# silencht/SG-SLAM

Hardware: AMD Instinct MI355X
Metric: tracked frames/sec (640x480 RGB-D) (higher is better)
Workload: dtype u8/f32(bf16x3 matrix products)/f64

## Files before the change

### include/sgx_debug.h

```cpp
#ifndef SGX_DEBUG_H
#define SGX_DEBUG_H
#include "sgx.h"
#ifdef __cplusplus
extern "C" {
#endif

int sgx_orb_debug_level_geometry(const sgx_orb *h, int level, int32_t *w, int32_t *hgt, int32_t *stride);
int sgx_orb_debug_set_unfused_pyramid(int on);
int sgx_orb_debug_read_level(sgx_orb *h, int frame, int level, uint8_t *dst );
int sgx_orb_debug_read_candidates(sgx_orb *h, int frame, int level, int32_t *x, int32_t *y, int32_t *score, int cap, int *n);
int sgx_debug_flow_affine_batch_dev(int batch, int cap, const sgx_keypoint *d_keys, const int32_t *d_n, const float *d_A, const float *d_shift, const float *d_boxes,
                                    int max_boxes, float *d_prev_xy, void *stream);
int sgx_pose_opt_debug_set_threads(int threads_per_frame);
int sgx_ba_debug_last_plan(int32_t plan[4]);
int sgx_ba_debug_set_init(int mode);
int sgx_ba_debug_set_jobs(int host);
int sgx_ba_debug_set_solver(int mode);
int sgx_det_debug_read_blob(sgx_det *h, const char *blob_name, int image, float *dst, int cap, int *n);
int sgx_flow_debug_read_level(sgx_flow *h, int slot, int frame, int level, uint8_t *img);
int sgx_flow_debug_level_size(const sgx_flow *h, int level, int32_t *w, int32_t *hgt);
int sgx_pnp_debug_betas(int which, const double *L, const double *rho, double *betas);
int sgx_debug_corun_bf16(int blocks, int iters, int launches, void *stream);
int sgx_det_debug_detection_output(sgx_det *h, const float *loc, const float *conf, int batch, sgx_det_result *results);
int sgx_det_debug_continued(sgx_det *h, int *count);
int sgx_det_debug_set_fusion(int on);
int sgx_det_debug_set_irb(int on);
int sgx_det_debug_set_block_fusion(int on);
int sgx_det_debug_set_gemm(int mode);
int sgx_det_debug_set_legacy_kernels(int on);
int sgx_det_debug_time_ops(sgx_det *h, const uint8_t *d_img, int pitch, int batch, int reps, float *ms, int cap, int *nops);
int sgx_det_debug_run_step(sgx_det *h, const uint8_t *d_img, int pitch, int batch, int step, int reps, void *stream);
int sgx_orb_debug_run_octree(sgx_orb *h, int level, const uint32_t *packed, int n, uint32_t *out_sel, int cap, int *nsel);

#ifdef __cplusplus
}
#endif
#endif
```

### sg_slam_amd/capi.py

```python
import ctypes as C
import numpy as np

KP_DTYPE = np.dtype([('x', 'f4'), ('y', 'f4'), ('size', 'f4'), ('angle', 'f4'), ('response', 'f4'),
                     ('octave', 'i4'), ('class_id', 'i4')])


class SgxError(RuntimeError):
    pass


class Camera(C.Structure):
    _fields_ = [('fx', C.c_float), ('fy', C.c_float), ('cx', C.c_float), ('cy', C.c_float), ('bf', C.c_float),
                ('min_x', C.c_float), ('max_x', C.c_float), ('min_y', C.c_float), ('max_y', C.c_float)]


class BaProblem(C.Structure):
    _fields_ = [('n_poses', C.c_int32), ('n_points', C.c_int32), ('n_edges', C.c_int32), ('poses', C.c_void_p), ('pose_fixed', C.c_void_p),
                ('points', C.c_void_p), ('edge_pose', C.c_void_p), ('edge_point', C.c_void_p), ('edge_obs', C.c_void_p), ('edge_info', C.c_void_p)]


class BaStats(C.Structure):
    _fields_ = [('iterations_first', C.c_int32), ('iterations_second', C.c_int32), ('free_poses', C.c_int32), ('reserved', C.c_int32),
                ('chi2_first', C.c_double), ('chi2_second', C.c_double)]


SGX_DET_MAX = 100


class Detection(C.Structure):
    _fields_ = [(k, C.c_float) for k in ('label', 'score', 'xmin', 'ymin', 'xmax', 'ymax')]


class Object2D(C.Structure):
    _fields_ = [('id', C.c_int32)] + [(k, C.c_float) for k in ('prob', 'x', 'y', 'w', 'h')]


class DetResult(C.Structure):
    _fields_ = [('n_raw', C.c_int32), ('raw', Detection * SGX_DET_MAX), ('n_objects', C.c_int32), ('objects', Object2D * SGX_DET_MAX),
                ('have_dynamic_for_mapping', C.c_int32), ('have_dynamic_for_rm_feature', C.c_int32),
                ('n_map_boxes', C.c_int32), ('map_boxes', Object2D * SGX_DET_MAX), ('n_rm_boxes', C.c_int32), ('rm_boxes', Object2D * SGX_DET_MAX)]


class FlowConfig(C.Structure):
    _fields_ = [('width', C.c_int32), ('height', C.c_int32), ('max_batch', C.c_int32), ('win_size', C.c_int32), ('max_level', C.c_int32),
                ('max_count', C.c_int32), ('epsilon', C.c_double)]


class TrackerConfig(C.Structure):
    _fields_ = [('streams', C.c_int32), ('width', C.c_int32), ('height', C.c_int32), ('nfeatures', C.c_int32), ('scale_factor', C.c_float), ('nlevels', C.c_int32),
                ('ini_th_fast', C.c_int32), ('min_th_fast', C.c_int32), ('cam', Camera), ('depth_map_factor', C.c_float), ('th_projection', C.c_float),
                ('local_map', C.c_int32), ('dynamic_mask', C.c_int32), ('max_boxes', C.c_int32), ('pipelined', C.c_int32)]


class OrbConfig(C.Structure):
    _fields_ = [('nfeatures', C.c_int32), ('scale_factor', C.c_float), ('nlevels', C.c_int32),
                ('ini_th_fast', C.c_int32), ('min_th_fast', C.c_int32), ('width', C.c_int32),
                ('height', C.c_int32), ('max_batch', C.c_int32)]


SYMBOLS = [
    'sgx_version', 'sgx_status_string', 'sgx_orb_create', 'sgx_orb_destroy', 'sgx_orb_keypoint_capacity', 'sgx_orb_get_tables',
    'sgx_orb_extract_batch_dev', 'sgx_orb_extract', 'sgx_orb_last_status', 'sgx_profile_enable', 'sgx_profile_num_classes', 'sgx_profile_class_name',
    'sgx_profile_read', 'sgx_match_project_frame_batch_dev', 'sgx_match_project_frame', 'sgx_match_project_local_batch_dev',
    'sgx_match_project_local', 'sgx_frame_stereo_from_rgbd_batch_dev', 'sgx_frame_unproject_batch_dev', 'sgx_frame_make_map_points_batch_dev',
    'sgx_frame_merge_matches_batch_dev', 'sgx_pose_optimization_batch_dev', 'sgx_pose_optimization', 'sgx_frame_motion_model_batch_dev',
    'sgx_local_bundle_adjustment', 'sgx_bundle_adjustment', 'sgx_det_create', 'sgx_det_destroy', 'sgx_det_info', 'sgx_det_detect',
    'sgx_det_detect_batch_dev', 'sgx_det_forward_batch_dev', 'sgx_frame_compact_keys_batch_dev', 'sgx_frame_gray_from_color_batch_dev',
    'sgx_det_gemm_mode', 'sgx_det_plan_step', 'sgx_dynamic_mask_batch_dev', 'sgx_tracker_create', 'sgx_tracker_destroy',
    'sgx_tracker_keypoint_capacity', 'sgx_tracker_record_bytes', 'sgx_tracker_set_initial_pose', 'sgx_tracker_step_dev', 'sgx_tracker_host_buffers',
    'sgx_tracker_step_host', 'sgx_tracker_wait_inputs', 'sgx_tracker_sync', 'sgx_tracker_read', 'sgx_tracker_snapshot_pose_dev',
    'sgx_tracker_snapshot_boxes_dev', 'sgx_tracker_pack_records_dev', 'sgx_tracker_frame_dev', 'sgx_tracker_extractor', 'sgx_flow_create',
    'sgx_dist_unique_id', 'sgx_dist_create', 'sgx_dist_destroy', 'sgx_dist_world', 'sgx_dist_gather_records',
    'sgx_flow_destroy', 'sgx_flow_reset', 'sgx_flow_levels', 'sgx_flow_lk_batch_dev', 'sgx_flow_lk', 'sgx_fundamental_ransac_batch_dev',
    'sgx_find_fundamental_mat', 'sgx_hamming_matrix', 'sgx_hamming_matrix_dev', 'sgx_match_search_for_triangulation', 'sgx_match_search_by_bow',
    'sgx_match_search_by_bow_kf', 'sgx_match_fuse_search', 'sgx_match_project_keyframe', 'sgx_match_fuse_search_sim3',
    'sgx_triangulate_new_map_points', 'sgx_mappoint_update_normal_and_depth', 'sgx_mappoint_distinctive_descriptors', 'sgx_sim3_solver_create',
    'sgx_sim3_solver_set_ransac_parameters', 'sgx_sim3_solver_iterate', 'sgx_sim3_solver_get_estimate', 'sgx_sim3_solver_destroy',
    'sgx_match_search_for_initialization', 'sgx_voc_load', 'sgx_voc_create', 'sgx_voc_info', 'sgx_voc_destroy', 'sgx_voc_transform',
    'sgx_voc_transform_batch_dev', 'sgx_voc_score', 'sgx_match_project_sim3', 'sgx_match_search_by_sim3', 'sgx_optimize_sim3',
    'sgx_optimize_essential_graph', 'sgx_correct_map_points', 'sgx_undistort_points', 'sgx_frame_undistort_stereo_rgbd_batch_dev', 'sgx_frame_image_bounds',
    'sgx_tracker_set_distortion', 'sgx_tracker_frame_keys_un_dev', 'sgx_pnp_solver_create', 'sgx_pnp_solver_set_ransac_parameters', 'sgx_pnp_solver_iterate',
    'sgx_pnp_solver_get_estimate', 'sgx_pnp_solver_destroy', 'sgx_pnp_batch_create', 'sgx_pnp_batch_set_dev', 'sgx_pnp_batch_iterate_dev', 'sgx_pnp_batch_destroy',
]
TAP_SYMBOLS = [
    'sgx_orb_debug_level_geometry', 'sgx_orb_debug_set_unfused_pyramid', 'sgx_orb_debug_read_level', 'sgx_orb_debug_read_candidates',
    'sgx_orb_debug_run_octree', 'sgx_pose_opt_debug_set_threads', 'sgx_ba_debug_set_solver', 'sgx_ba_debug_set_jobs', 'sgx_ba_debug_set_init', 'sgx_ba_debug_last_plan', 'sgx_det_debug_read_blob',
    'sgx_det_debug_detection_output', 'sgx_det_debug_continued', 'sgx_debug_flow_affine_batch_dev', 'sgx_det_debug_set_fusion', 'sgx_det_debug_set_legacy_kernels',
    'sgx_det_debug_set_block_fusion', 'sgx_det_debug_set_irb', 'sgx_det_debug_set_gemm', 'sgx_det_debug_time_ops', 'sgx_det_debug_run_step', 'sgx_flow_debug_read_level',
    'sgx_flow_debug_level_size', 'sgx_debug_corun_bf16', 'sgx_pnp_debug_betas',
]


def _vp(x):
    if x is None:
        return None
    if isinstance(x, int):
        return C.c_void_p(x)
    if hasattr(x, 'data_ptr'):
        return C.c_void_p(x.data_ptr())
    return x.ctypes.data_as(C.c_void_p)


class SgxLib:
    def __init__(self, path):
        self.path = path
        self.dll = C.CDLL(path)
        d = self.dll
        d.sgx_version.restype = C.c_char_p
        d.sgx_status_string.restype = C.c_char_p
        d.sgx_status_string.argtypes = [C.c_int]
        d.sgx_orb_create.argtypes = [C.POINTER(OrbConfig), C.POINTER(C.c_void_p)]
        d.sgx_orb_destroy.argtypes = [C.c_void_p]
        d.sgx_orb_destroy.restype = None
        d.sgx_orb_keypoint_capacity.argtypes = [C.c_void_p]
        d.sgx_orb_get_tables.argtypes = [C.c_void_p] + [C.c_void_p] * 5
        d.sgx_orb_extract_batch_dev.argtypes = [C.c_void_p, C.c_void_p, C.c_int, C.c_int, C.c_void_p, C.c_void_p,
                                                C.c_void_p, C.c_int, C.c_void_p]
        d.sgx_orb_extract.argtypes = [C.c_void_p, C.c_void_p, C.c_int, C.c_void_p, C.c_void_p, C.c_int, C.POINTER(C.c_int)]
        d.sgx_orb_last_status.argtypes = [C.c_void_p, C.c_void_p]

        d.sgx_profile_enable.argtypes = [C.c_int]
        d.sgx_profile_class_name.restype = C.c_char_p
        d.sgx_profile_class_name.argtypes = [C.c_int]
        d.sgx_profile_read.argtypes = [C.c_void_p, C.c_void_p, C.c_int]

        vp = C.c_void_p
        d.sgx_match_project_frame_batch_dev.argtypes = [C.c_int, C.c_int] + [vp] * 13 + [C.POINTER(Camera), vp, C.c_int, C.c_float, C.c_int, C.c_int, vp, vp, vp]
        d.sgx_match_project_frame.argtypes = [C.c_int] + [vp] * 4 + [C.c_int] + [vp] * 7 + [C.POINTER(Camera), vp, C.c_int, C.c_float, C.c_int, C.c_int, vp, vp]
        d.sgx_frame_stereo_from_rgbd_batch_dev.argtypes = [C.c_int, C.c_int, vp, vp, vp, C.c_int, C.c_int, C.c_float, C.c_float, vp, vp, vp]
        d.sgx_frame_unproject_batch_dev.argtypes = [C.c_int, C.c_int, vp, vp, vp, vp, C.POINTER(Camera), vp, vp, vp]
        d.sgx_pose_optimization_batch_dev.argtypes = [C.c_int, C.c_int, vp, vp, vp, vp, vp, vp, C.c_int, vp, C.c_int, C.POINTER(Camera), vp, vp, vp, vp]
        d.sgx_pose_optimization.argtypes = [C.c_int, vp, vp, vp, vp, vp, C.c_int, C.POINTER(Camera), vp, vp, vp]
        d.sgx_frame_motion_model_batch_dev.argtypes = [C.c_int, vp, vp, vp, vp, vp]
        d.sgx_local_bundle_adjustment.argtypes = [C.POINTER(BaProblem), C.POINTER(Camera), vp, vp, C.POINTER(BaStats)]
        d.sgx_bundle_adjustment.argtypes = [C.POINTER(BaProblem), C.POINTER(Camera), C.c_int, vp, C.c_int, C.POINTER(BaStats)]
        d.sgx_det_create.argtypes = [C.c_char_p, vp, C.c_size_t, C.c_int, C.c_int, C.c_int, C.c_float, C.c_float, C.POINTER(vp)]
        d.sgx_det_destroy.argtypes = [vp]; d.sgx_det_destroy.restype = None
        d.sgx_det_info.argtypes = [vp, C.POINTER(C.c_int32), C.POINTER(C.c_int32), C.POINTER(C.c_int32), C.POINTER(C.c_double)]
        d.sgx_det_detect.argtypes = [vp, vp, C.c_int, C.c_int, C.POINTER(DetResult)]
        d.sgx_det_detect_batch_dev.argtypes = [vp, vp, C.c_int, C.c_int, vp, vp, vp, C.c_int, vp, vp]
        d.sgx_det_forward_batch_dev.argtypes = [vp, vp, C.c_int, C.c_int, C.POINTER(vp), C.POINTER(vp), vp]
        d.sgx_det_gemm_mode.argtypes = [vp]
        d.sgx_tracker_create.argtypes = [C.POINTER(TrackerConfig), vp, C.POINTER(vp)]
        d.sgx_tracker_destroy.argtypes = [vp]; d.sgx_tracker_destroy.restype = None
        d.sgx_tracker_keypoint_capacity.argtypes = [vp]
        d.sgx_tracker_record_bytes.argtypes = [vp]
        d.sgx_tracker_set_initial_pose.argtypes = [vp, vp]
        d.sgx_tracker_step_dev.argtypes = [vp, vp, C.c_int, vp, vp, C.c_int, vp]
        d.sgx_tracker_host_buffers.argtypes = [vp, C.c_int, C.POINTER(vp), C.POINTER(C.c_int), C.POINTER(vp)]
        d.sgx_tracker_step_host.argtypes = [vp, C.c_int, C.c_int]
        d.sgx_tracker_sync.argtypes = [vp]
        d.sgx_tracker_wait_inputs.argtypes = [vp, C.c_int]
        d.sgx_tracker_read.argtypes = [vp] * 10
        d.sgx_tracker_snapshot_pose_dev.argtypes = [vp, vp]
        d.sgx_tracker_snapshot_boxes_dev.argtypes = [vp, C.c_int, vp, vp]
        d.sgx_tracker_pack_records_dev.argtypes = [vp, vp, vp]
        d.sgx_dist_unique_id.argtypes = [vp]
        d.sgx_dist_create.argtypes = [vp, C.c_int, C.c_int, C.POINTER(vp)]
        d.sgx_dist_destroy.argtypes = [vp]; d.sgx_dist_destroy.restype = None
        d.sgx_dist_world.argtypes = [vp, C.POINTER(C.c_int32), C.POINTER(C.c_int32)]
        d.sgx_dist_gather_records.argtypes = [vp, vp, C.c_size_t, vp, C.c_int, vp]
        d.sgx_tracker_frame_dev.argtypes = [vp] + [C.POINTER(vp)] * 6
        d.sgx_tracker_extractor.argtypes = [vp]; d.sgx_tracker_extractor.restype = vp
        d.sgx_det_plan_step.argtypes = [vp, C.c_int, C.c_char_p, C.c_int]
        d.sgx_dynamic_mask_batch_dev.argtypes = [C.c_int, C.c_int, vp, vp, vp, vp, vp, vp, C.c_int, vp, vp]
        d.sgx_frame_gray_from_color_batch_dev.argtypes = [C.c_int, C.c_int, C.c_int, vp, C.c_int, C.c_int, C.c_int, vp, C.c_int, vp]
        d.sgx_frame_compact_keys_batch_dev.argtypes = [C.c_int, C.c_int, vp, vp, vp, vp, vp, C.c_int, vp, vp, vp, vp]
        d.sgx_match_project_local.argtypes = [C.c_int] + [vp] * 5 + [C.c_int] + [vp] * 7 + [C.POINTER(Camera), vp, C.c_int, C.c_float, C.c_float, C.c_float, C.c_float, vp, vp, vp]
        d.sgx_match_project_local_batch_dev.argtypes = [C.c_int, C.c_int] + [vp] * 6 + [C.c_int] + [vp] * 8 + [C.POINTER(Camera), vp, C.c_int, C.c_float, C.c_float, C.c_float, C.c_float, vp, vp, vp, vp]
        d.sgx_undistort_points.argtypes = [C.c_int, vp, vp, vp, C.c_int, vp]
        d.sgx_frame_undistort_stereo_rgbd_batch_dev.argtypes = [C.c_int, C.c_int, vp, vp, vp, C.c_int, C.POINTER(Camera), vp, C.c_int, C.c_int, C.c_float, vp, vp, vp, vp]
        d.sgx_frame_image_bounds.argtypes = [C.c_int, C.c_int, vp, vp, C.c_int, C.POINTER(Camera)]
        d.sgx_tracker_set_distortion.argtypes = [vp, vp, C.c_int, C.POINTER(Camera)]
        d.sgx_tracker_frame_keys_un_dev.argtypes = [vp, C.POINTER(vp)]
        d.sgx_frame_make_map_points_batch_dev.argtypes = [C.c_int, C.c_int, C.c_int] + [vp] * 7 + [C.c_int] + [vp] * 7
        d.sgx_frame_merge_matches_batch_dev.argtypes = [C.c_int, C.c_int] + [vp] * 10
        d.sgx_flow_create.argtypes = [C.POINTER(FlowConfig), C.POINTER(vp)]
        d.sgx_flow_destroy.argtypes = [vp]; d.sgx_flow_destroy.restype = None
        d.sgx_flow_reset.argtypes = [vp]
        d.sgx_flow_levels.argtypes = [vp]
        d.sgx_flow_lk_batch_dev.argtypes = [vp, vp, C.c_int, C.c_int, vp, vp, C.c_int, vp, vp, C.POINTER(C.c_int32), vp]
        d.sgx_flow_lk.argtypes = [vp, vp, vp, C.c_int, vp, C.c_int, vp, vp]
        d.sgx_fundamental_ransac_batch_dev.argtypes = [C.c_int, C.c_int] + [vp] * 6 + [C.c_int, C.c_double, C.c_double, vp, vp, vp, vp]
        d.sgx_find_fundamental_mat.argtypes = [vp, vp, C.c_int, C.c_double, C.c_double, vp, vp, vp]
        d.sgx_hamming_matrix.argtypes = [vp, C.c_int, vp, C.c_int, vp]
        d.sgx_optimize_essential_graph.argtypes = [C.c_int, vp, vp, C.c_int, vp, vp, vp, C.c_int, C.c_int, vp, vp]
        d.sgx_correct_map_points.argtypes = [C.c_int, vp, vp, C.c_int, vp, vp, vp]
        d.sgx_optimize_sim3.argtypes = [C.c_int] + [vp] * 9 + [C.c_float, C.c_int, vp, vp, vp]
        d.sgx_match_project_keyframe.argtypes = [C.c_int] + [vp] * 4 + [C.c_int] + [vp] * 6 + [C.POINTER(Camera), vp, C.c_int, C.c_float, C.c_float, C.c_int, C.c_int, vp, vp]
        d.sgx_match_search_by_bow.argtypes = [C.c_int] + [vp] * 4 + [C.c_int] + [vp] * 3 + [C.c_float, C.c_int, vp, vp]
        d.sgx_match_fuse_search_sim3.argtypes = [C.c_int, vp, vp, vp, C.c_int] + [vp] * 6 + [vp, vp, C.c_int, C.c_float, C.c_float, vp, vp, vp]
        d.sgx_match_project_sim3.argtypes = [C.c_int, vp, vp, vp, vp, C.c_int] + [vp] * 6 + [vp, vp, C.c_int, C.c_float, C.c_int, vp, vp]
        d.sgx_match_search_by_sim3.argtypes = ([C.c_int] + [vp] * 8) * 2 + [vp, vp, C.c_int, C.c_float, C.c_float, vp, vp, C.c_float, vp, vp]
        d.sgx_match_search_for_initialization.argtypes = [C.c_int, vp, vp, C.c_int, vp, vp, vp, C.c_int, C.c_float, C.c_int, vp, vp, vp]
        d.sgx_sim3_solver_create.argtypes = [C.c_int] + [vp] * 6 + [C.c_int, C.c_uint, vp]
        d.sgx_sim3_solver_set_ransac_parameters.argtypes = [vp, C.c_double, C.c_int, C.c_int]
        d.sgx_sim3_solver_iterate.argtypes = [vp, C.c_int] + [vp] * 7
        d.sgx_sim3_solver_get_estimate.argtypes = [vp] * 5
        d.sgx_sim3_solver_destroy.argtypes = [vp]; d.sgx_sim3_solver_destroy.restype = None
        d.sgx_pnp_solver_create.argtypes = [C.c_int] + [vp] * 4 + [C.c_uint, vp]
        d.sgx_pnp_solver_set_ransac_parameters.argtypes = [vp, C.c_double, C.c_int, C.c_int, C.c_int, C.c_float, C.c_float]
        d.sgx_pnp_solver_iterate.argtypes = [vp, C.c_int] + [vp] * 7
        d.sgx_pnp_solver_get_estimate.argtypes = [vp] * 6
        d.sgx_pnp_solver_destroy.argtypes = [vp]; d.sgx_pnp_solver_destroy.restype = None
        d.sgx_pnp_batch_create.argtypes = [C.c_int, C.c_int, vp]
        d.sgx_pnp_batch_set_dev.argtypes = [vp, C.c_int] + [vp] * 8
        d.sgx_pnp_batch_iterate_dev.argtypes = [vp, C.c_int, vp, C.c_int, vp, vp, vp, vp]
        d.sgx_pnp_batch_destroy.argtypes = [vp]; d.sgx_pnp_batch_destroy.restype = None
        d.sgx_mappoint_update_normal_and_depth.argtypes = [C.c_int] + [vp] * 6 + [C.c_int, vp, vp, vp]
        d.sgx_mappoint_distinctive_descriptors.argtypes = [C.c_int, vp, vp, vp, vp]
        d.sgx_triangulate_new_map_points.argtypes = [C.c_int, vp] + [C.c_int] + [vp] * 5 + [C.c_int] + [vp] * 5 + [vp, vp, vp, C.c_int, vp, vp, vp]
        d.sgx_voc_load.argtypes = [C.c_char_p, vp]
        d.sgx_voc_create.argtypes = [C.c_int] * 5 + [vp] * 5
        d.sgx_voc_info.argtypes = [vp] * 7
        d.sgx_voc_destroy.argtypes = [vp]; d.sgx_voc_destroy.restype = None
        d.sgx_voc_transform.argtypes = [vp, C.c_int, vp, C.c_int, vp, vp, vp, vp, vp]
        d.sgx_voc_transform_batch_dev.argtypes = [vp, vp, C.c_size_t, vp, C.c_int, C.c_int, C.c_int, vp, vp, vp, vp]
        d.sgx_voc_score.argtypes = [vp, C.c_int, vp, vp, C.c_int, vp, vp, vp]
        d.sgx_match_search_by_bow_kf.argtypes = [C.c_int] + [vp] * 4 + [C.c_int] + [vp] * 4 + [C.c_float, C.c_int, vp, vp]
        d.sgx_match_fuse_search.argtypes = [C.c_int] + [vp] * 4 + [C.c_int] + [vp] * 6 + [C.POINTER(Camera), vp, vp, C.c_int, C.c_float, C.c_float, vp, vp, vp]
        d.sgx_hamming_matrix_dev.argtypes = [vp, C.c_int, vp, C.c_int, vp, vp]
        d.sgx_match_search_for_triangulation.argtypes = [C.c_int] + [vp] * 6 + [C.c_int] + [vp] * 6 + [vp, C.POINTER(Camera), vp, vp, C.c_int, C.c_int, C.c_int, vp, vp]

        self.has_taps = hasattr(d, 'sgx_det_debug_read_blob')
        if self.has_taps:
            d.sgx_orb_debug_level_geometry.argtypes = [C.c_void_p, C.c_int] + [C.POINTER(C.c_int32)] * 3
            d.sgx_orb_debug_read_level.argtypes = [C.c_void_p, C.c_int, C.c_int, C.c_void_p]
            d.sgx_orb_debug_read_candidates.argtypes = [C.c_void_p, C.c_int, C.c_int, C.c_void_p, C.c_void_p, C.c_void_p, C.c_int, C.POINTER(C.c_int)]
            d.sgx_orb_debug_run_octree.argtypes = [C.c_void_p, C.c_int, C.c_void_p, C.c_int, C.c_void_p, C.c_int, C.POINTER(C.c_int)]
            d.sgx_orb_debug_set_unfused_pyramid.argtypes = [C.c_int]
            d.sgx_pose_opt_debug_set_threads.argtypes = [C.c_int]
            d.sgx_ba_debug_set_solver.argtypes = [C.c_int]
            d.sgx_ba_debug_set_jobs.argtypes = [C.c_int]
            d.sgx_ba_debug_set_init.argtypes = [C.c_int]
            d.sgx_ba_debug_last_plan.argtypes = [C.c_void_p]
            d.sgx_det_debug_detection_output.argtypes = [vp, vp, vp, C.c_int, C.POINTER(DetResult)]
            d.sgx_det_debug_continued.argtypes = [vp, C.POINTER(C.c_int)]
            d.sgx_det_debug_read_blob.argtypes = [vp, C.c_char_p, C.c_int, vp, C.c_int, C.POINTER(C.c_int)]
            for nm in ('fusion', 'legacy_kernels', 'block_fusion', 'irb', 'gemm'):
                getattr(d, 'sgx_det_debug_set_' + nm).argtypes = [C.c_int]
            d.sgx_det_debug_time_ops.argtypes = [vp, vp, C.c_int, C.c_int, C.c_int, vp, C.c_int, C.POINTER(C.c_int)]
            d.sgx_det_debug_run_step.argtypes = [vp, vp, C.c_int, C.c_int, C.c_int, C.c_int, vp]
            d.sgx_debug_flow_affine_batch_dev.argtypes = [C.c_int, C.c_int, vp, vp, vp, vp, vp, C.c_int, vp, vp]
            d.sgx_flow_debug_read_level.argtypes = [vp, C.c_int, C.c_int, C.c_int, vp]
            d.sgx_debug_corun_bf16.argtypes = [C.c_int, C.c_int, C.c_int, vp]
            d.sgx_pnp_debug_betas.argtypes = [C.c_int, vp, vp, vp]
            d.sgx_flow_debug_level_size.argtypes = [vp, C.c_int, C.POINTER(C.c_int32), C.POINTER(C.c_int32)]

    def tap(self, name):
        if not self.has_taps:
            raise SgxError(f'{name}: {self.path} is the product build and has no test taps; use tests/taps/libsgx_taps.so (make -C sg_slam_amd/csrc taps)')
        return getattr(self.dll, name)

    def version(self):
        return self.dll.sgx_version().decode()

    def check(self, rc, what=''):
        if rc != 0:
            raise SgxError(f'{what}: {self.dll.sgx_status_string(rc).decode()} ({rc})')

    def profile_enable(self, on=True):
        self.check(self.dll.sgx_profile_enable(int(on)))

    def profile_read(self, reset=True):
        n = self.dll.sgx_profile_num_classes()
        ms = np.zeros(n, 'f4'); cnt = np.zeros(n, 'i4')
        self.check(self.dll.sgx_profile_read(_vp(ms), _vp(cnt), int(reset)), 'sgx_profile_read')
        return {self.dll.sgx_profile_class_name(k).decode(): (float(ms[k]), int(cnt[k])) for k in range(n)}
```

### sg_slam_amd/csrc/sgx_det.cpp

```cpp
#include "sgx_block.h"
#include "sgx_det_block.h"
#include "sgx_det_irb.h"
#include "sgx_det_bf16.h"
#include "sgx_det_hrb.h"
#include "sgx_prof.h"
#include "../../include/sgx.h"
#ifdef SGX_DEBUG_TAPS
#include "../../include/sgx_debug.h"
#endif
#include <math.h>
#include <stdio.h>
#include <stdlib.h>
#include <string.h>
#include <algorithm>
#include <map>
#include <memory>
#include <sstream>
#include <string>
#include <vector>


namespace {
struct Layer {
    std::string type, name;
    std::vector<std::string> ins, outs;
    std::map<int, double> p;
    std::map<int, std::vector<float>> pa;
    int geti(int k, int d) const { auto it = p.find(k); return it == p.end() ? d : (int)it->second; }
    float getf(int k, float d) const { auto it = p.find(k); return it == p.end() ? d : (float)it->second; }
};
struct Blob { int c = 0, h = 0, w = 0; size_t n = 0; float *d = nullptr; bool scalar = false; float sval = 0.f; int alias = -1; };
enum OpKind { OP_PW, OP_KXK, OP_BINARY, OP_UNARY, OP_PERMUTE_INTO, OP_COPY_INTO, OP_SOFTMAX, OP_FUSED_BLOCK, OP_IRB, OP_SE_GATE };
struct EpiStep { int op, src; float a, b; int tensor; };
struct Op {
    OpKind kind; int in0 = -1, in1 = -1, out = -1;
    std::vector<EpiStep> epi; int hwc = 0, hwc_off = 0; bool dead = false; std::string name;
    int inc = 0, outc = 0, H = 0, W = 0, Ho = 0, Wo = 0, k = 1, stride = 1, pad = 0, depthwise = 0, act = 0; float lo = 0, hi = 0;
    std::vector<float> hw, hb;
    float *wt = nullptr, *bias = nullptr, *wtT = nullptr, *wtP = nullptr; int ldw = 0;
    int bop = 0; int off = 0; int rows = 0, C = 0;
    void *wS = nullptr;
    int res_blob = -1;
    SgxFusedBlk fb;
    SgxSeGate sg;
    SgxIrb irb; int irb_out2_blob = -1;
};
}

#ifndef SGX_DET_GRAPH_EXECS
#define SGX_DET_GRAPH_EXECS 1
#endif
#ifndef SGX_DET_FORK_LANES
#define SGX_DET_FORK_LANES 1
#endif

#ifndef SGX_DET_GEMM_DEFAULT
#define SGX_DET_GEMM_DEFAULT 1
#endif
struct DetSwitches {
    int fuse = 1, legacy = 0, block_fusion = 0;
    int irb = 1;
    int gemm = SGX_DET_GEMM_DEFAULT;
    int block2 = 1, block2_se = 1, hrb = 1, hrb_pick = 0, fb2_tile = -1, fb_dbg = 0;
    int irb_mask = 0xff;
    int irb_g = 0, irb_nbuf = 0, irb_split = 0, irb_minhw = 0, irb_stagger = 1, irb_w1lds = 0, irb3 = 0, irb3_dbg = 0, irb_a3 = 0, irb_dual = 1, se_gate = 1;
    int prefuse = 1, xcd = 1;
    int stem_words = 13824, dw2 = 1, dw3 = 0, dw_budget = 8192, pw3_mink = 64, pw3_force = 0, pw2_direct = 1;
    int no_graph = 0, fork_lanes = SGX_DET_FORK_LANES, graph_execs = SGX_DET_GRAPH_EXECS, skip_output = 0;
    int out_single = 0;
};

struct sgx_det {
    int T = 300, max_batch = 1, W = 0, H = 0;
    int pre_fused = 0;
    DetSwitches sw;
    float det_th = 0.9f, dyn_th = 0.01f;
    std::vector<Layer> layers;
    std::map<std::string, int> blob_id;
    std::vector<Blob> blobs;
    std::vector<Op> ops;
    std::vector<void *> dev;
    std::vector<float> priors;
    int num_priors = 0, num_class = 21, nms_top_k = 300, keep_top_k = 100; float nms_th = 0.45f, conf_th = 0.01f, dvar[4] = {0.1f, 0.1f, 0.2f, 0.2f};
    int loc_blob = -1, conf_blob = -1;
    SgxDetTab *d_xt = nullptr, *d_yt = nullptr; uint8_t *d_img = nullptr;
    float *d_priors = nullptr, *d_cls_rows = nullptr; int *d_cls_count = nullptr; sgx_det_result *d_results = nullptr;
    int *d_cls_ncut = nullptr, *d_cls_cont = nullptr; uint32_t *d_cls_next = nullptr, *d_sstar = nullptr;
    int last_out_batch = 0;
    double gmac = 0;
#ifndef SGX_EMU
    std::map<int, std::vector<hipGraphExec_t>> graphs;
    std::map<int, unsigned> graph_turn;
    std::vector<hipStream_t> fork_streams;
    std::vector<hipEvent_t> fork_events;
#endif
    ~sgx_det() {
#ifndef SGX_EMU
        for (auto &g : graphs) for (hipGraphExec_t e : g.second) (void)hipGraphExecDestroy(e);
        for (hipEvent_t e : fork_events) (void)hipEventDestroy(e);
        for (hipStream_t q : fork_streams) (void)hipStreamDestroy(q);
#endif
        for (void *p : dev) (void)hipFree(p);
    }
    template <class Tp> int alloc(Tp **p, size_t n) { void *q = nullptr; if (hipMalloc(&q, (n ? n : 1) * sizeof(Tp)) != hipSuccess) return SGX_ERR_NOMEM; dev.push_back(q); *p = (Tp *)q; return SGX_OK; }
    template <class Tp, class Pp> int upload(Pp *dst, const Tp *src, size_t n) { Tp *d = nullptr; if (alloc(&d, n)) return SGX_ERR_NOMEM; *dst = (Pp)d; return hipMemcpy(d, src, n * sizeof(Tp), hipMemcpyHostToDevice) == hipSuccess ? SGX_OK : SGX_ERR_DEVICE; }
    template <class Tp, class Pp> int upload(Pp *dst, const std::vector<Tp> &v) { return upload(dst, v.data(), v.size()); }
    int resolve(int id) const { while (blobs[id].alias >= 0) id = blobs[id].alias; return id; }
    bool is_output(int id) const { return id == loc_blob || id == conf_blob; }
};

static thread_local int g_det_fuse = 1, g_det_block_fusion = 0, g_det_legacy = 0;
static thread_local int g_det_irb = -1, g_det_gemm = -1;
SGX_TAP int sgx_det_debug_set_fusion(int on) { g_det_fuse = on ? 1 : 0; return SGX_OK; }
SGX_TAP int sgx_det_debug_set_legacy_kernels(int on) { g_det_legacy = on ? 1 : 0; return SGX_OK; }
SGX_TAP int sgx_det_debug_set_block_fusion(int on) { g_det_block_fusion = on ? 1 : 0; return SGX_OK; }
SGX_TAP int sgx_det_debug_set_irb(int on) { g_det_irb = on < 0 ? -1 : (on > 2 ? 2 : on); return SGX_OK; }
SGX_TAP int sgx_det_debug_set_gemm(int mode) { g_det_gemm = mode < 0 ? -1 : (mode ? 1 : 0); return SGX_OK; }
extern "C" int sgx_det_gemm_mode(const sgx_det *h) { return h ? h->sw.gemm : -1; }

static DetSwitches det_switches()
{
    auto env = [](const char *name, int &v) { if (const char *e = sgx_getenv(name)) v = atoi(e); };
    DetSwitches s;
    s.fuse = g_det_fuse; s.legacy = g_det_legacy; s.block_fusion = (g_det_block_fusion || sgx_getenv("SGX_DET_BLOCK_FUSION")) ? 1 : 0;
    env("SGX_DET_IRB", s.irb); if (g_det_irb >= 0) s.irb = g_det_irb;
#ifdef SGX_EMU
    s.gemm = 0;
#endif
    if (const char *e = sgx_getenv("SGX_DET_GEMM")) if (*e) s.gemm = (!strcmp(e, "f32") || !strcmp(e, "0")) ? 0 : 1;
    if (g_det_gemm >= 0) s.gemm = g_det_gemm;
    if (s.legacy) s.gemm = 0;
    env("SGX_DET_BLOCK2", s.block2); env("SGX_DET_BLOCK2_SE", s.block2_se); env("SGX_DET_HRB", s.hrb); env("SGX_HRB_PICK", s.hrb_pick); env("SGX_FB2_TILE", s.fb2_tile); env("SGX_FB_DBG", s.fb_dbg);
    env("SGX_DET_IRB_MASK", s.irb_mask); env("SGX_IRB_G", s.irb_g); env("SGX_IRB_NBUF", s.irb_nbuf); env("SGX_IRB_SPLIT", s.irb_split); env("SGX_IRB_MINHW", s.irb_minhw);
    env("SGX_IRB_STAGGER", s.irb_stagger); env("SGX_IRB_W1LDS", s.irb_w1lds); env("SGX_DET_IRB3", s.irb3); env("SGX_IRB3_DBG", s.irb3_dbg); env("SGX_DET_IRB_A3", s.irb_a3);
    env("SGX_DET_IRB_DUAL", s.irb_dual); env("SGX_DET_SE_GATE", s.se_gate); env("SGX_DET_PREFUSE", s.prefuse); env("SGX_DET_XCD", s.xcd);
    env("SGX_DET_STEM_WORDS", s.stem_words); env("SGX_DW2", s.dw2); env("SGX_DW3", s.dw3); env("SGX_DW_BUDGET", s.dw_budget);
    env("SGX_PW3_MINK", s.pw3_mink); env("SGX_PW3_FORCE", s.pw3_force); env("SGX_PW2_DIRECT", s.pw2_direct);
    s.no_graph = sgx_getenv("SGX_DET_NO_GRAPH") != nullptr; env("SGX_DET_FORK", s.fork_lanes); env("SGX_DET_EXECS", s.graph_execs);
    s.skip_output = sgx_getenv("SGX_DET_SKIP_OUTPUT") != nullptr;
    s.out_single = sgx_getenv("SGX_DET_OUT_SINGLE") != nullptr;
    return s;
}

struct Stem2Geom { int nbx4, pitch4, RB, nbands; size_t lds; };
static Stem2Geom stem2_geom(const sgx_det *h, const Op &op)
{
    Stem2Geom g;
    g.nbx4 = (op.Wo + 3) / 4; g.pitch4 = ((g.nbx4 - 1) * 4 * op.stride + 3 * op.stride + op.k + 3) & ~3;
    const int words = h->sw.stem_words;
    g.RB = std::max(1, std::min(op.Ho, ((words / (3 * g.pitch4)) - 3) / 2 + 1));
    g.nbands = (op.Ho + g.RB - 1) / g.RB;
    g.lds = (size_t)3 * ((g.RB - 1) * 2 + 3) * g.pitch4 * 4;
    return g;
}
static SgxEpi make_epi(const sgx_det *h, const Op &op, size_t tpitch);
static bool stem2_ok(const sgx_det *h, const Op &op)
{
    if (op.kind != OP_KXK || !h->sw.dw2 || h->sw.legacy || op.depthwise || !op.wtT || op.outc > 16 || op.inc != 3 || op.k != 3 || op.stride != 2) return false;
    const Stem2Geom g = stem2_geom(h, op);
    if (!(3 * 5 * g.pitch4 * 4 <= 65536 && g.pitch4 < 4096)) return false;
    const int mode = make_epi(h, op, 0).mode;
    return mode == SGX_EMODE_NONE || mode == SGX_EMODE_ACT || mode == SGX_EMODE_HSWISH;
}

static int parse_param(const char *text, std::vector<Layer> &layers)
{
    std::istringstream is(text);
    std::string line;
    if (!std::getline(is, line) || atoi(line.c_str()) != 7767517) return SGX_ERR_INVALID;
    if (!std::getline(is, line)) return SGX_ERR_INVALID;
    while (std::getline(is, line)) {
        std::istringstream ls(line);
        Layer L; int nin = 0, nout = 0;
        if (!(ls >> L.type >> L.name >> nin >> nout)) continue;
        for (int i = 0; i < nin; i++) { std::string s; ls >> s; L.ins.push_back(s); }
        for (int i = 0; i < nout; i++) { std::string s; ls >> s; L.outs.push_back(s); }
        std::string kv;
        while (ls >> kv) {
            const size_t eq = kv.find('=');
            if (eq == std::string::npos) continue;
            const int k = atoi(kv.substr(0, eq).c_str());
            const std::string v = kv.substr(eq + 1);
            if (k <= -23300) {
                std::vector<float> arr; std::istringstream vs(v); std::string tok; bool first = true;
                while (std::getline(vs, tok, ',')) { if (first) { first = false; continue; } arr.push_back((float)atof(tok.c_str())); }
                L.pa[-k - 23300] = arr;
            } else L.p[k] = atof(v.c_str());
        }
        layers.push_back(L);
    }
    return layers.empty() ? SGX_ERR_INVALID : SGX_OK;
}

static void build_tab(int s, int d, std::vector<SgxDetTab> &t)
{
    t.resize(d);
    const double scale = (double)s / d;
    for (int i = 0; i < d; i++) {
        float f = (float)((i + 0.5) * scale - 0.5);
        int si = (int)floorf(f); f -= si;
        if (si < 0) { si = 0; f = 0.f; }
        if (si >= s - 1) { si = s - 2; f = 1.f; }
        t[i].o = (short)si; t[i].a0 = (short)lrintf((1.f - f) * 2048); t[i].a1 = (short)lrintf(f * 2048); t[i].pad = 0;
    }
}

extern "C" void sgx_det_destroy(sgx_det *h) { delete h; }

namespace {
struct Loader {
    sgx_det *h; const uint8_t *bp; size_t bin_bytes, bo = 0;
    std::vector<float> prior_boxes, prior_vars;
    int blob(const std::string &n) { auto it = h->blob_id.find(n); if (it != h->blob_id.end()) return it->second; h->blob_id[n] = (int)h->blobs.size(); h->blobs.push_back(Blob()); return (int)h->blobs.size() - 1; }
    void same_shape_op(Op &op, const Layer &L, const Blob &A) { const int oid = blob(L.outs[0]); Blob &ob = h->blobs[oid]; ob = A; ob.alias = -1; ob.d = nullptr; op.out = oid; op.name = L.name; h->ops.push_back(op); }
    int conv(const Layer &L, int in0, const Blob &A);
    void priorbox(const Layer &L, const Blob &A);
    int run();
};

std::vector<float> pair_interleave(const std::vector<float> &w, int C, int kk)
{
    std::vector<float> p((size_t)C * kk); for (int m = 0; m < C; m++) for (int t = 0; t < kk; t++) p[((size_t)(m >> 1) * kk + t) * 2 + (m & 1)] = w[(size_t)m * kk + t]; return p;
}
int upload_se_interleaved(sgx_det *h, const Op &d, const Op &e, const float **wq1p, const float **wq2p)
{
    const int Cq = d.outc, Co = d.inc;
    std::vector<float> p1((size_t)Cq * Co), p2((size_t)Co * Cq);
    for (int j = 0; j < Cq; j++) for (int k = 0; k < Co; k++) p1[((size_t)(j >> 1) * Co + k) * 2 + (j & 1)] = d.hw[(size_t)j * Co + k];
    for (int co = 0; co < Co; co++) for (int j = 0; j < Cq; j++) p2[((size_t)j * (Co / 2) + (co >> 1)) * 2 + (co & 1)] = e.hw[(size_t)co * Cq + j];
    const int rc = h->upload(wq1p, p1);
    return rc ? rc : h->upload(wq2p, p2);
}

int Loader::conv(const Layer &L, int in0, const Blob &A)
{
    Op op; const int outc = L.geti(0, 0), k = L.geti(1, 1), stride = L.geti(3, 1), pad = L.geti(4, 0), wsize = L.geti(6, 0), group = L.geti(7, 1);
    const int inc = A.c;
    if (L.geti(2, 1) != 1 || (group != 1 && group != inc) || wsize != outc * (inc / group) * k * k) return SGX_ERR_UNSUPPORTED;
    if (bo + 4 + (size_t)wsize * 4 + (L.geti(5, 0) ? (size_t)outc * 4 : 0) > bin_bytes) return SGX_ERR_INVALID;
    uint32_t flag; memcpy(&flag, bp + bo, 4); bo += 4;
    if (flag != 0) return SGX_ERR_UNSUPPORTED;
    op.hw.resize(wsize); memcpy(op.hw.data(), bp + bo, (size_t)wsize * 4); bo += (size_t)wsize * 4;
    op.hb.assign(outc, 0.f);
    if (L.geti(5, 0)) { memcpy(op.hb.data(), bp + bo, (size_t)outc * 4); bo += (size_t)outc * 4; }
    int rc = h->upload(&op.wt, op.hw); if (rc) return rc;
    if ((rc = h->upload(&op.bias, op.hb))) return rc;
    const bool pw = (k == 1 && group == 1 && stride == 1 && pad == 0), stem = (group == 1 && k > 1 && outc <= 16);
    if (pw || stem) {
        const int kk = inc * k * k, ldo = pw ? ((outc + 31) / 32) * 32 + 128 : 16;
        op.ldw = ldo;
        std::vector<float> wT((size_t)(pw ? ((kk + 31) / 32) * 32 : kk) * ldo, 0.f);
        for (int o = 0; o < outc; o++) for (int q = 0; q < kk; q++) wT[(size_t)q * ldo + o] = op.hw[(size_t)o * kk + q];
        if ((rc = h->upload(&op.wtT, wT))) return rc;
        if (pw && h->sw.gemm == 1) {
            std::vector<unsigned short> ws((size_t)((kk + 15) / 16) * 6 * ldo * 8);
            sgx_split_weights_bf16x3(op.hw.data(), outc, kk, ldo, ws.data());
            if ((rc = h->upload(&op.wS, ws))) return rc;
        }
    }
#ifdef SGX_DEBUG_TAPS
    if (group == inc && group != 1 && (outc & 1) == 0 && inc == outc && (rc = h->upload(&op.wtP, pair_interleave(op.hw, outc, k * k)))) return rc;
#endif
    op.inc = inc; op.outc = outc; op.H = A.h; op.W = A.w; op.k = k; op.stride = stride; op.pad = pad; op.depthwise = group != 1;
    op.Ho = (A.h + 2 * pad - k) / stride + 1; op.Wo = (A.w + 2 * pad - k) / stride + 1;
    op.kind = pw ? OP_PW : OP_KXK;
    op.in0 = in0;
    h->gmac += (double)op.Ho * op.Wo * wsize * 1e-9;
    const int oid = blob(L.outs[0]); Blob &ob = h->blobs[oid]; ob = Blob(); ob.c = outc; ob.h = op.Ho; ob.w = op.Wo; ob.n = (size_t)outc * op.Ho * op.Wo;
    op.out = oid; op.name = L.name;
    h->ops.push_back(op);
    return SGX_OK;
}

void Loader::priorbox(const Layer &L, const Blob &A)
{
    const int T = h->T;
    const std::vector<float> mins = L.pa.count(0) ? L.pa.at(0) : std::vector<float>(), maxs = L.pa.count(1) ? L.pa.at(1) : std::vector<float>(), ars = L.pa.count(2) ? L.pa.at(2) : std::vector<float>();
    const int flip = L.geti(7, 1), clip = L.geti(8, 0); const float offset = L.getf(13, 0.f);
    const float step_w = (float)T / (float)A.w, step_h = (float)T / (float)A.h;
    const float var[4] = { L.getf(3, .1f), L.getf(4, .1f), L.getf(5, .2f), L.getf(6, .2f) };
    auto add = [&](float cx, float cy, float bw, float bh) {
        float bx[4] = { (cx - bw * 0.5f) / T, (cy - bh * 0.5f) / T, (cx + bw * 0.5f) / T, (cy + bh * 0.5f) / T };
        for (int q = 0; q < 4; q++) { prior_boxes.push_back(clip ? std::min(std::max(bx[q], 0.f), 1.f) : bx[q]); prior_vars.push_back(var[q]); }
    };
    for (int i = 0; i < A.h; i++) for (int j = 0; j < A.w; j++) {
        const float cx = ((float)j + offset) * step_w, cy = ((float)i + offset) * step_h;
        for (size_t kk = 0; kk < mins.size(); kk++) {
            const float ms = mins[kk]; add(cx, cy, ms, ms);
            if (!maxs.empty()) { const float s = sqrtf(ms * maxs[kk]); add(cx, cy, s, s); }
            for (float ar : ars) { const float sq = sqrtf(ar); add(cx, cy, ms * sq, ms / sq); if (flip) add(cx, cy, ms / sq, ms * sq); }
        }
    }
    blob(L.outs[0]);
}

int Loader::run()
{
    const int B = h->max_batch, T = h->T;
    for (const Layer &L : h->layers) {
        if (L.type == "Input") { Blob &b = h->blobs[blob(L.outs[0])]; b.c = 3; b.h = T; b.w = T; b.n = (size_t)3 * T * T; if (h->alloc(&b.d, b.n * B)) return SGX_ERR_NOMEM; continue; }
        if (L.type == "MemoryData") {
            const int n = L.geti(0, 0) * std::max(L.geti(1, 1), 1) * std::max(L.geti(2, 1), 1);
            if (n != 1 || bo + 4 > bin_bytes) return SGX_ERR_UNSUPPORTED;
            Blob &b = h->blobs[blob(L.outs[0])]; b.scalar = true; memcpy(&b.sval, bp + bo, 4); bo += 4; b.n = 1; continue;
        }
        if (L.type == "Split") { const int src = h->resolve(blob(L.ins[0])); for (const std::string &o : L.outs) { const int id = blob(o); h->blobs[id] = h->blobs[src]; h->blobs[id].alias = src; } continue; }
        const int in0 = h->resolve(blob(L.ins[0]));
        const Blob A = h->blobs[in0];
        if (L.type == "Convolution" || L.type == "ConvolutionDepthWise") { const int rc = conv(L, in0, A); if (rc) return rc; continue; }
        if (L.type == "ReLU" || L.type == "Clip") {
            Op op; op.kind = OP_UNARY; op.in0 = in0; op.act = L.type == "ReLU" ? SGX_ACT_RELU : SGX_ACT_CLIP; op.lo = L.getf(0, 0.f); op.hi = L.getf(1, 0.f);
            same_shape_op(op, L, A); continue;
        }
        if (L.type == "BinaryOp") {
            const int in1 = h->resolve(blob(L.ins[1]));
            Op op; op.kind = OP_BINARY; op.in0 = in0; op.in1 = in1; op.bop = L.geti(0, 0);
            if (op.bop != 0 && op.bop != 2 && op.bop != 3) return SGX_ERR_UNSUPPORTED;
            if (!h->blobs[in1].scalar && h->blobs[in1].n != A.n) return SGX_ERR_UNSUPPORTED;
            same_shape_op(op, L, A); continue;
        }
        const int raw_in = blob(L.ins[0]);
        if (L.type == "Permute") { if (L.geti(0, 0) != 3) return SGX_ERR_UNSUPPORTED; const int oid = blob(L.outs[0]); h->blobs[oid] = A; h->blobs[oid].alias = raw_in; h->blobs[oid].sval = 1.f;  continue; }
        if (L.type == "Flatten") { const int oid = blob(L.outs[0]); h->blobs[oid] = A; h->blobs[oid].sval = 0.f; h->blobs[oid].alias = raw_in; continue; }
        if (L.type == "PriorBox") { priorbox(L, A); continue; }
        if (L.type == "Concat") {
            if (L.name == "mbox_priorbox") { blob(L.outs[0]); continue; }
            size_t total = 0; for (const std::string &i : L.ins) total += h->blobs[h->resolve(blob(i))].n;
            const int oid = blob(L.outs[0]); Blob &ob = h->blobs[oid]; ob.c = 1; ob.h = 1; ob.w = (int)total; ob.n = total;
            int off = 0;
            for (const std::string &i : L.ins) {
                int id = blob(i); bool hwc = false; while (h->blobs[id].alias >= 0) { if (h->blobs[id].sval == 1.f) hwc = true; id = h->blobs[id].alias; }
                Op op; op.kind = hwc ? OP_PERMUTE_INTO : OP_COPY_INTO; op.in0 = id; op.out = oid; op.off = off; op.C = h->blobs[id].c; op.rows = h->blobs[id].h * h->blobs[id].w;
                op.name = L.name; h->ops.push_back(op); off += (int)h->blobs[id].n;
            }
            continue;
        }
        if (L.type == "Reshape") { const int oid = blob(L.outs[0]); h->blobs[oid] = A; h->blobs[oid].alias = raw_in; h->blobs[oid].w = L.geti(0, 1); h->blobs[oid].h = (int)(A.n / L.geti(0, 1)); continue; }
        if (L.type == "Softmax") {
            Op op; op.kind = OP_SOFTMAX; op.in0 = in0; op.C = h->blobs[blob(L.ins[0])].w; op.rows = (int)(A.n / op.C);
            if (op.C < 1 || op.C > SGX_SOFTMAX_MAXC) return SGX_ERR_UNSUPPORTED;
            same_shape_op(op, L, A); continue;
        }
        if (L.type == "DetectionOutput") {
            h->loc_blob = h->resolve(blob(L.ins[0])); h->conf_blob = h->resolve(blob(L.ins[1]));
            h->num_class = L.geti(0, 21); h->nms_th = L.getf(1, 0.45f); h->nms_top_k = L.geti(2, 300); h->keep_top_k = L.geti(3, 100); h->conf_th = L.getf(4, 0.01f);
            h->dvar[0] = L.getf(5, .1f); h->dvar[1] = L.getf(6, .1f); h->dvar[2] = L.getf(7, .2f); h->dvar[3] = L.getf(8, .2f);
            continue;
        }
        return SGX_ERR_UNSUPPORTED;
    }
    if (h->loc_blob < 0 || h->conf_blob < 0) return SGX_ERR_INVALID;
    h->num_priors = (int)prior_boxes.size() / 4;
    h->priors = prior_boxes; h->priors.insert(h->priors.end(), prior_vars.begin(), prior_vars.end());
    return SGX_OK;
}

struct EpiClass { int mode = SGX_EMODE_GENERIC; float c1 = 0.f, lo = 0.f, hi = INFINITY, c2 = 1.f; int i0 = -1, i1 = -1, t0 = -1, t1 = -1; };
template <class Step> EpiClass classify_epi(const Step *e, size_t n)
{
    EpiClass r;
    auto is = [&](size_t i, int opc, int src) { return i < n && e[i].op == opc && (opc == SGX_EOP_CLIP || opc == SGX_EOP_RELU || e[i].src == src); };
    if (n == 0) r.mode = SGX_EMODE_NONE;
    else if (n == 1 && is(0, SGX_EOP_RELU, 0)) { r.mode = SGX_EMODE_ACT; r.lo = 0.f; r.hi = INFINITY; }
    else if (n == 1 && is(0, SGX_EOP_CLIP, 0)) { r.mode = SGX_EMODE_ACT; r.lo = e[0].a; r.hi = e[0].b; }
    else if (n == 1 && is(0, SGX_EOP_ADD, SGX_ESRC_TENSOR)) { r.mode = SGX_EMODE_ADD_T; r.i1 = 0; }
    else if (n == 4 && is(0, SGX_EOP_ADD, SGX_ESRC_CONST) && is(1, SGX_EOP_CLIP, 0) && is(2, SGX_EOP_MUL, SGX_ESRC_ROOT) && is(3, SGX_EOP_DIV, SGX_ESRC_CONST)) {
        r.mode = SGX_EMODE_HSWISH; r.c1 = e[0].a; r.lo = e[1].a; r.hi = e[1].b; r.c2 = e[3].a;
    } else if ((n == 4 || n == 5) && is(0, SGX_EOP_ADD, SGX_ESRC_CONST) && is(1, SGX_EOP_CLIP, 0) && is(2, SGX_EOP_DIV, SGX_ESRC_CONST) && is(3, SGX_EOP_MUL, SGX_ESRC_TENSOR) &&
               (n == 4 || is(4, SGX_EOP_ADD, SGX_ESRC_TENSOR))) {
        r.mode = n == 4 ? SGX_EMODE_GATE : SGX_EMODE_GATE_ADD; r.c1 = e[0].a; r.lo = e[1].a; r.hi = e[1].b; r.c2 = e[2].a; r.i0 = 3; if (n == 5) r.i1 = 4;
    }
    return r;
}
EpiClass classify(const std::vector<EpiStep> &e) { EpiClass r = classify_epi(e.data(), e.size()); if (r.i0 >= 0) r.t0 = e[r.i0].tensor; if (r.i1 >= 0) r.t1 = e[r.i1].tensor; return r; }

SgxFusedBlk make_fused_blk(const Op &a, const Op &bq, const Op &c, const EpiClass &ca, const EpiClass &cb)
{
    SgxFusedBlk fb; memset(&fb, 0, sizeof fb);
    fb.Cin = a.inc; fb.Cmid = a.outc; fb.Cout = c.outc; fb.K = bq.k; fb.stride = bq.stride; fb.pad = bq.pad; fb.H = a.H; fb.W = a.W; fb.Ho = bq.Ho; fb.Wo = bq.Wo;
    fb.lo1 = ca.lo; fb.hi1 = ca.hi; fb.lo2 = cb.lo; fb.hi2 = cb.hi;
    fb.w1 = a.wt; fb.b1 = a.bias; fb.wd = bq.wt; fb.bd = bq.bias; fb.w2 = c.wt; fb.b2 = c.bias;
    return fb;
}
void set_tiles(SgxFusedBlk &fb) { fb.tiles_x = (fb.Wo + fb.TOW - 1) / fb.TOW; fb.tiles_y = (fb.Ho + fb.TOH - 1) / fb.TOH; }
Op make_block_op(const Op &a, const Op &bq, const Op &c, const SgxFusedBlk &fb, int out, int res, const std::string &name)
{
    Op f; f.kind = OP_FUSED_BLOCK; f.in0 = a.in0; f.out = out; f.name = name; f.fb = fb; f.res_blob = res;
    f.inc = a.inc; f.outc = c.outc; f.H = a.H; f.W = a.W; f.Ho = bq.Ho; f.Wo = bq.Wo; f.k = bq.k; f.stride = bq.stride;
    return f;
}

struct Planner {
    sgx_det *h; const DetSwitches &sw; std::vector<Op> &ops; const int nops, B;
    std::vector<int> R;
    explicit Planner(sgx_det *h_) : h(h_), sw(h_->sw), ops(h_->ops), nops((int)h_->ops.size()), B(h_->max_batch) {}
    bool fb2_on() const { return sw.block2 != 0 && !sw.legacy && sw.fuse; }
    void readers(int id, std::vector<int> &r, bool all = false) const
    {
        r.clear();
        for (int i = 0; i < nops; i++) {
            const Op &o = ops[i];
            if (o.dead) continue;
            bool rd = o.in0 == id || (o.kind == OP_BINARY && o.in1 == id && !h->blobs[id].scalar);
            if (all) {
                rd = rd || o.res_blob == id;
                for (const EpiStep &st : o.epi) rd = rd || st.tensor == id;
            }
            if (rd) r.push_back(i);
        }
    }
    void readers_all(int id, std::vector<int> &r) const { readers(id, r, true); }
    int fuse_epilogues(), fuse_blocks(), fuse_irb(), fuse_se_gates(), merge_dual_heads();
    int fuse_block_fb1(int ai, int bi, int ci, const EpiClass &ca, const EpiClass &cb, int res);
    struct IrbMatch { int ai = -1, bi = -1, ci = -1, di = -1, ei = -1, out_blob = -1, res_blob = -1; EpiClass ca, cb, cc, cd, ce; };
    bool match_irb(int bi, IrbMatch &m);
    int fuse_block2_se(const IrbMatch &m, bool *taken);
    bool irb_geometry(const IrbMatch &m, SgxIrb &ib) const;
};

int Planner::fuse_epilogues()
{
    std::vector<int> producer(h->blobs.size(), -2);
    producer[h->resolve(h->blob_id.at("input"))] = -1;
    for (int i = 0; i < nops; i++) if (ops[i].kind != OP_PERMUTE_INTO && ops[i].kind != OP_COPY_INTO) producer[ops[i].out] = i;
    for (int ci = 0; ci < nops; ci++) {
        Op &cv = ops[ci];
        if (cv.kind != OP_PW && cv.kind != OP_KXK) continue;
        const int root = cv.out;
        int cur = root, root_extra = -1;
        std::vector<EpiStep> steps; std::vector<int> absorbed;
        while ((int)steps.size() < SGX_EPI_MAX) {
            if (h->is_output(cur)) break;
            readers(cur, R);
            int next = -1;
            if (R.size() == 1) next = R[0];
            else if (cur == root && R.size() == 2 && steps.empty()) { next = std::min(R[0], R[1]); root_extra = std::max(R[0], R[1]); }
            else break;
            const Op &e = ops[next];
            EpiStep st; st.a = 0; st.b = 0; st.tensor = -1; st.src = SGX_ESRC_CONST;
            if (e.kind == OP_UNARY) { st.op = e.act == SGX_ACT_RELU ? SGX_EOP_RELU : SGX_EOP_CLIP; st.a = e.lo; st.b = e.hi; }
            else if (e.kind == OP_BINARY) {
                if (e.in0 == cur && e.in1 == cur) break;
                const bool first = e.in0 == cur;
                const int other = first ? e.in1 : e.in0;
                const int fwd = e.bop == 0 ? SGX_EOP_ADD : e.bop == 2 ? SGX_EOP_MUL : SGX_EOP_DIV;
                st.op = first ? fwd : (e.bop == 3 ? SGX_EOP_RDIV : fwd);
                if (h->blobs[other].scalar) { st.src = SGX_ESRC_CONST; st.a = h->blobs[other].sval; }
                else if (other == root && cur != root) { st.src = SGX_ESRC_ROOT; }
                else if (producer[other] >= -1 && producer[other] < ci && h->blobs[other].n == h->blobs[root].n) { st.src = SGX_ESRC_TENSOR; st.tensor = other; }
                else break;
            } else break;
            steps.push_back(st); absorbed.push_back(next); cur = e.out;
        }
        if (root_extra >= 0 && std::find(absorbed.begin(), absorbed.end(), root_extra) == absorbed.end()) { steps.clear(); absorbed.clear(); cur = root; }
        if (!steps.empty()) {
            cv.epi = steps; cv.out = cur;
            for (int a : absorbed) ops[a].dead = true;
            producer[cur] = ci;
        }
        if (cv.kind == OP_PW) {
            bool tens = false; for (const EpiStep &st : cv.epi) tens = tens || st.src == SGX_ESRC_TENSOR;
            readers(cv.out, R);
            if (!tens && R.size() == 1 && ops[R[0]].kind == OP_PERMUTE_INTO && !h->is_output(cv.out)) {
                cv.hwc = 1; cv.hwc_off = ops[R[0]].off; cv.out = ops[R[0]].out; ops[R[0]].dead = true;
            }
        }
    }
    return SGX_OK;
}

int Planner::fuse_blocks()
{
    const bool fb1_on = sw.block_fusion && !sw.legacy;
    if (!fb1_on && !fb2_on()) return SGX_OK;
    for (int ai = 0; ai < nops; ai++) {
        Op &a = ops[ai];
        if (a.dead || a.kind != OP_PW || a.hwc) continue;
        const EpiClass ca = classify(a.epi);
        if (ca.mode != SGX_EMODE_ACT) continue;
        readers(a.out, R); if (R.size() != 1) continue;
        const int bi = R[0]; Op &bq = ops[bi];
        const EpiClass cb = classify(bq.epi);
        if (bq.kind != OP_KXK || !bq.depthwise || (bq.k != 3 && bq.k != 5) || cb.mode != SGX_EMODE_ACT) continue;
        readers(bq.out, R); if (R.size() != 1) continue;
        const int ci = R[0]; Op &c = ops[ci];
        if (c.kind != OP_PW || c.hwc || c.in0 != bq.out) continue;
        const EpiClass cc = classify(c.epi);
        if (cc.mode != SGX_EMODE_NONE && cc.mode != SGX_EMODE_ADD_T) continue;
        if (a.outc != bq.outc || c.inc != bq.outc) continue;
        if (h->is_output(a.out) || h->is_output(bq.out)) continue;
        const int v2 = sgx_fb2_variant(a.inc, c.outc, bq.k, bq.stride, 0, sw.fb2_tile);
        if (fb2_on() && v2 && (a.outc % sgx_fb2_cm(v2)) == 0 && c.wtT && bq.pad == bq.k / 2) {
            SgxFusedBlk fb = make_fused_blk(a, bq, c, ca, cb);
            fb.v2 = v2; fb.w2t = c.wtT; fb.ldw2 = c.ldw;
            sgx_fb2_tile(v2, &fb.TOH, &fb.TOW);
            const int rc = h->upload(&fb.wd2, pair_interleave(bq.hw, fb.Cmid, bq.k * bq.k)); if (rc) return rc;
            if (sw.hrb && h->sw.gemm == 1 && a.wS && c.wS && sgx_hrb_variant(fb.Cin, fb.Cmid, fb.Cout, fb.K, fb.stride, 0, cc.t1 >= 0, fb.lo1, fb.lo2, sw.hrb_pick, &fb.TOH, &fb.TOW, &fb.hrb_occ)) {
                fb.hrb = 1; fb.w1S = a.wS; fb.ld1S = a.ldw; fb.w2S = c.wS; fb.ld2S = c.ldw;
            }
            set_tiles(fb);
            ops[ci] = make_block_op(a, bq, c, fb, c.out, cc.t1, a.name + "+" + bq.name + "+" + c.name); a.dead = true; bq.dead = true;
            continue;
        }
        if (fb1_on) { const int rc = fuse_block_fb1(ai, bi, ci, ca, cb, cc.t1); if (rc) return rc; }
    }
    return SGX_OK;
}

int Planner::fuse_block_fb1(int ai, int bi, int ci, const EpiClass &ca, const EpiClass &cb, int res)
{
    Op &a = ops[ai], &bq = ops[bi], &c = ops[ci];
    if ((a.inc & 1) || (a.outc & 1) || a.inc > 64 || c.outc > 64) return SGX_OK;
    SgxFusedBlk fb = make_fused_blk(a, bq, c, ca, cb);
    const int ncb = (fb.Cout + 31) / 32, nch = (fb.Cmid + 31) / 32;
    auto tile = [&](SgxFusedBlk &t, int th, int tw) {
        t.TOH = th; t.TOW = tw; t.TIH = (th - 1) * fb.stride + fb.K; t.TIW = (tw - 1) * fb.stride + fb.K;
        t.NPI = ((t.TIH * t.TIW + 31) / 32) * 32; t.NPO = ((th * tw + 31) / 32) * 32; t.CMR = std::min(32, fb.Cmid); t.ES = t.NPI + 4;
    };
    double best = 1e30; int bth = 0, btw = 0;
    for (int th = 1; th <= 16; th++) for (int tw = 4; tw <= 40; tw++) {
        SgxFusedBlk t = fb; tile(t, th, tw);
        if (ncb * (t.NPO / 32) > 8 || sgx_fb_lds_floats(t) * 4 > 52 * 1024 || fb.Cout * th * tw > 64 * 1024 || t.NPI >= (1 << 12) || th * tw >= (1 << 12)) continue;
        const int txn = (fb.Wo + tw - 1) / tw, tyn = (fb.Ho + th - 1) / th;
        const double cost = (double)txn * tyn * (nch * ((t.NPI / 32) * (fb.Cin / 2.0) + (t.NPO / 32) * ncb * 16.0) * 64.0 / 4.0 + (double)fb.Cmid * th * tw * fb.K * fb.K * 4.0 / 256.0 * 2.0 + 3000.0);
        if (cost < best) { best = cost; bth = th; btw = tw; }
    }
    if (!bth) return SGX_OK;
    tile(fb, bth, btw); set_tiles(fb);
    fb.m_tiw = sgx_magic(fb.TIW); fb.m_tow = sgx_magic(btw); fb.m_npo = sgx_magic(bth * btw); fb.m_kk = sgx_magic(fb.K * fb.K);
    fb.dbg = sw.fb_dbg;
    ops[ci] = make_block_op(a, bq, c, fb, c.out, res, a.name + "+" + bq.name + "+" + c.name); a.dead = true; bq.dead = true;
    return SGX_OK;
}

bool Planner::match_irb(int bi, IrbMatch &m)
{
    const Op &bq = ops[bi];
    if (bq.dead || bq.kind != OP_KXK || !bq.depthwise || (bq.k != 3 && bq.k != 5) || (bq.stride != 1 && bq.stride != 2) || bq.pad != bq.k / 2 || bq.inc != bq.outc) return false;
    m = IrbMatch(); m.bi = bi; m.ca.mode = m.cd.mode = m.ce.mode = SGX_EMODE_NONE;
    m.cb = classify(bq.epi);
    if (m.cb.mode != SGX_EMODE_ACT && m.cb.mode != SGX_EMODE_HSWISH) return false;
    if (h->is_output(bq.out)) return false;
    readers_all(bq.out, R); if (R.size() != 1) return false;
    m.ci = R[0]; const Op &c = ops[m.ci];
    if (c.kind != OP_PW || c.in0 != bq.out || !c.wtT || c.inc != bq.outc || (c.inc & 1)) return false;
    m.cc = classify(c.epi);
    if (m.cc.mode != SGX_EMODE_NONE && m.cc.mode != SGX_EMODE_ADD_T) return false;
    if (c.hwc && m.cc.mode != SGX_EMODE_NONE) return false;
    for (int i = 0; i < nops; i++) if (!ops[i].dead && ops[i].kind == OP_PW && ops[i].out == bq.in0 && !ops[i].hwc) m.ai = i;
    if (m.ai >= 0) {
        readers_all(bq.in0, R);
        m.ca = classify(ops[m.ai].epi);
        if (R.size() != 1 || !ops[m.ai].wtT || (ops[m.ai].inc & 1) || (m.ca.mode != SGX_EMODE_ACT && m.ca.mode != SGX_EMODE_HSWISH) || h->is_output(bq.in0)) { m.ai = -1; m.ca = EpiClass(); m.ca.mode = SGX_EMODE_NONE; }
    }
    m.out_blob = c.out; m.res_blob = m.cc.mode == SGX_EMODE_ADD_T ? m.cc.t1 : -1;
    if (!c.hwc && m.cc.mode == SGX_EMODE_NONE && !h->is_output(c.out)) {
        readers_all(c.out, R);
        if (R.size() == 2) {
            for (int q = 0; q < 2; q++) {
                const Op &d = ops[R[q]], &e = ops[R[1 - q]];
                if (d.kind != OP_PW || e.kind != OP_PW || d.in0 != c.out || d.hwc || e.hwc || !d.wtT || !e.wtT || e.in0 != d.out || (d.outc & 1) || (d.inc & 1)) continue;
                m.cd = classify(d.epi); m.ce = classify(e.epi);
                if (m.cd.mode != SGX_EMODE_ACT || (m.ce.mode != SGX_EMODE_GATE && m.ce.mode != SGX_EMODE_GATE_ADD) || m.ce.t0 != c.out || e.outc != c.outc) continue;
                std::vector<int> R2; readers_all(d.out, R2); if (R2.size() != 1) continue;
                m.di = R[q]; m.ei = R[1 - q]; m.out_blob = e.out; m.res_blob = m.ce.mode == SGX_EMODE_GATE_ADD ? m.ce.t1 : -1;
            }
        }
    }
    return true;
}

int Planner::fuse_block2_se(const IrbMatch &m, bool *taken)
{
    *taken = false;
    if (!(fb2_on() && sw.block2_se && sw.irb == 1 && m.ai >= 0 && m.di >= 0 && !ops[m.ci].hwc && m.ca.mode == SGX_EMODE_ACT && m.cb.mode == SGX_EMODE_ACT)) return SGX_OK;
    const Op &a = ops[m.ai], &bq = ops[m.bi], &c = ops[m.ci], &d = ops[m.di], &e = ops[m.ei];
    const int v2 = sgx_fb2_variant(a.inc, c.outc, bq.k, bq.stride, d.outc, sw.fb2_tile);
    const bool res = m.res_blob >= 0;
    int h_toh = 0, h_tow = 0, h_occ = 0;
    const bool hrb_ok = sw.hrb && h->sw.gemm == 1 && a.wS && c.wS && d.wS && e.wS && bq.pad == bq.k / 2 &&
                        sgx_hrb_variant(a.inc, a.outc, c.outc, bq.k, bq.stride, d.outc, res, m.ca.lo, m.cb.lo, sw.hrb_pick, &h_toh, &h_tow, &h_occ);
    if (!((hrb_ok || (v2 && (a.outc % sgx_fb2_cm(v2)) == 0)) && a.outc == bq.outc && d.inc == c.outc && e.inc == d.outc)) return SGX_OK;
    SgxFusedBlk fb = make_fused_blk(a, bq, c, m.ca, m.cb);
    fb.v2 = v2; fb.w2t = c.wtT; fb.ldw2 = c.ldw;
    if (v2) sgx_fb2_tile(v2, &fb.TOH, &fb.TOW);
    fb.Cq = d.outc; fb.qlo = m.cd.lo; fb.qhi = m.cd.hi; fb.gc1 = m.ce.c1; fb.glo = m.ce.lo; fb.ghi = m.ce.hi; fb.gc2 = m.ce.c2;
    fb.wq1 = d.wt; fb.bq1 = d.bias; fb.wq2 = e.wt; fb.bq2 = e.bias;
    int rc = h->upload(&fb.wd2, pair_interleave(bq.hw, fb.Cmid, bq.k * bq.k)); if (rc) return rc;
    if ((rc = upload_se_interleaved(h, d, e, &fb.wq1p, &fb.wq2p))) return rc;
    if (hrb_ok) {
        fb.hrb = 1; fb.TOH = h_toh; fb.TOW = h_tow; fb.hrb_occ = h_occ;
        fb.w1S = a.wS; fb.ld1S = a.ldw; fb.w2S = c.wS; fb.ld2S = c.ldw; fb.wq1S = d.wS; fb.ldq1S = d.ldw; fb.wq2S = e.wS; fb.ldq2S = e.ldw;
    }
    set_tiles(fb);
    const Op f = make_block_op(a, bq, c, fb, m.out_blob, m.res_blob, a.name + "+" + bq.name + "+" + c.name + "+" + d.name + "+" + e.name);
    ops[m.ai].dead = true; ops[m.bi].dead = true; ops[m.ci].dead = true; ops[m.di].dead = true; ops[m.ei] = f;
    *taken = true;
    return SGX_OK;
}

bool Planner::irb_geometry(const IrbMatch &m, SgxIrb &ib) const
{
    const Op &bq = ops[m.bi];
    const size_t lds_max = 160 * 1024; const int kkp = SGX_IRB_KKP(bq.k), max_px = 384;
    auto lds_of = [&](int g, int oh, int nb) { const int planeT = ((g * ((oh - 1) * bq.stride + bq.k) * ib.Wp + 3) / 4) * 4; return (size_t)nb * 32 * (planeT + kkp) * 4; };
    int G = 0, OH = bq.Ho, nbands = 1, nbuf = 2;
    if (bq.Ho * bq.Wo < sw.irb_minhw) return false;
    const bool split = sw.irb_split > 0 && bq.Ho * bq.Wo >= sw.irb_split;
    if (!split && bq.Ho * bq.Wo <= max_px && lds_of(1, bq.Ho, 1) <= lds_max) {
        G = std::min(std::max(1, max_px / (bq.Ho * bq.Wo)), bq.Ho * bq.Wo >= 64 ? 1 : 2);
        if (sw.irb_g > 0) G = std::min(std::max(1, max_px / (bq.Ho * bq.Wo)), sw.irb_g);
        while (G > 1 && lds_of(G, bq.Ho, 2) > lds_max) G--;
        nbuf = lds_of(G, bq.Ho, 2) <= lds_max ? 2 : 1;
    } else {
        G = 1; OH = std::max(1, std::min(split ? (bq.Ho + 1) / 2 : bq.Ho, max_px / bq.Wo));
        while (OH > 1 && lds_of(1, OH, 1) > lds_max) OH--;
        if (lds_of(1, OH, 1) > lds_max || OH * bq.Wo > 1024) return false;
        nbands = (bq.Ho + OH - 1) / OH; OH = (bq.Ho + nbands - 1) / nbands;
        nbuf = lds_of(1, OH, 2) <= lds_max ? 2 : 1;
    }
    if (sw.irb_nbuf == 1) nbuf = 1;
    ib.G = G; ib.OH = OH; ib.nbands = nbands; ib.nbuf = nbuf;
    ib.HpWp = ((OH - 1) * bq.stride + bq.k) * ib.Wp; ib.planeT = ((G * ib.HpWp + 3) / 4) * 4;
    const size_t big = (size_t)B * std::max(std::max(h->blobs[m.ai >= 0 ? ops[m.ai].in0 : bq.in0].n, h->blobs[m.out_blob].n), (size_t)1) * 4;
    return big < 0xFFFFFFFFull;
}

int Planner::fuse_irb()
{
    if (sw.irb == 0 || sw.legacy) return SGX_OK;
    IrbMatch m;
    for (int bi = 0; bi < nops; bi++) {
        if (!match_irb(bi, m)) continue;
        bool taken = false;
        int rc = fuse_block2_se(m, &taken); if (rc) return rc;
        if (taken) continue;
        Op &bq = ops[bi], &c = ops[m.ci];
        const int ai = m.ai, di = m.di, ei = m.ei;
        const bool head = c.hwc != 0;
        const int kind_bit = head ? 8 : (ai < 0 ? 4 : (bq.stride == 2 ? 2 : 1));
        if (!(sw.irb_mask & kind_bit)) continue;
        if (sw.irb == 1) {
            const int px = bq.Ho * bq.Wo;
            const bool win = head || (ai >= 0 && ops[ai].inc >= 40 && px >= 256 && px <= 400);
            if (!win) continue;
        }
        const int NT = (c.outc + 31) / 32, NQ = di >= 0 ? (ops[di].outc + 31) / 32 : 0;
        if (!sgx_irb_supported(bq.k, bq.stride, NT, NQ, ai >= 0, m.cb.mode == SGX_EMODE_HSWISH)) continue;
        if (ai >= 0 && m.ca.mode != m.cb.mode) continue;
        if (bq.outc % 8) continue;
        SgxIrb ib; memset(&ib, 0, sizeof ib);
        ib.Cin = ai >= 0 ? ops[ai].inc : bq.inc; ib.Cexp = bq.outc; ib.Cout = c.outc; ib.Cq = di >= 0 ? ops[di].outc : 0;
        ib.H = bq.H; ib.W = bq.W; ib.Ho = bq.Ho; ib.Wo = bq.Wo; ib.K = bq.k; ib.S = bq.stride; ib.pad = bq.pad;
        ib.Wp = bq.W + 2 * bq.pad;
        if (!irb_geometry(m, ib)) continue;
        ib.has_expand = ai >= 0; ib.stagger = sw.irb_stagger; ib.dbg = sw.irb3_dbg;
        const EpiClass &ca = m.ca, &cb = m.cb, &cd = m.cd, &ce = m.ce;
        if (ai >= 0) { ib.act1 = ca.mode; ib.a1c1 = ca.c1; ib.a1lo = ca.lo; ib.a1hi = ca.hi; ib.a1c2 = ca.c2; ib.w1T = ops[ai].wtT; ib.b1 = ops[ai].bias; ib.ld1 = ops[ai].ldw; ib.w1 = ops[ai].wt; }
        ib.act2 = cb.mode; ib.a2c1 = cb.c1; ib.a2lo = cb.lo; ib.a2hi = cb.hi; ib.a2c2 = cb.c2;
        ib.w2T = c.wtT; ib.b2 = c.bias; ib.ld2 = c.ldw; ib.w2 = c.wt; ib.wd = bq.wt; ib.bd = bq.bias;
        if (di >= 0) {
            ib.qlo = cd.lo; ib.qhi = cd.hi; ib.gc1 = ce.c1; ib.glo = ce.lo; ib.ghi = ce.hi; ib.gc2 = ce.c2;
            ib.wq1T = ops[di].wtT; ib.bq1 = ops[di].bias; ib.ldq1 = ops[di].ldw; ib.wq1 = ops[di].wt;
            ib.wq2T = ops[ei].wtT; ib.bq2 = ops[ei].bias; ib.ldq2 = ops[ei].ldw; ib.wq2 = ops[ei].wt;
        }
        ib.has_res = m.res_blob >= 0; ib.hwc = c.hwc; ib.hwc_off = c.hwc_off;
        if (ai >= 0 && sw.irb_w1lds) {
            ib.w1rows = (((ib.Cin >> 1) + 7) & ~7) * 2;
            if (sgx_irb_lds_bytes(ib) > (size_t)160 * 1024) ib.w1rows = 0;
        }
        {
            const int nqs = NQ == 0 ? 1 : (NQ == 2 ? 3 : (NT == 2 ? 1 : 2));
            const bool ok3 = sw.irb3 != 0 && h->sw.gemm == 1 && c.wS && (ai < 0 || ops[ai].wS) && (di < 0 || (ops[di].wS && ops[ei].wS && (ops[di].outc + 15) / 16 == nqs));
            ib.gemm = ok3 ? 1 : 0;
            const int a3 = sw.irb_a3;
            if (!ok3 && a3 && h->sw.gemm == 1 && ai >= 0 && ops[ai].wS) { ib.gemm = 2; ib.w1S = ops[ai].wS; }
            if (ib.gemm == 2 && a3 >= 2 && (a3 == 2 || bq.outc == a3)) {
                ib.ldS = ((bq.H * bq.W + 31) / 32) * 32;
                unsigned *sh = nullptr; if (h->alloc(&sh, (size_t)B * ((ops[ai].inc + 15) / 16) * 6 * ib.ldS * 4)) return SGX_ERR_NOMEM;
                ib.inS = sh;
            } else if (ib.gemm == 2 && a3 > 2 && bq.outc != a3) ib.gemm = 0;
            if (ok3) { ib.w2S = c.wS; ib.w1S = ai >= 0 ? ops[ai].wS : nullptr; ib.wq1S = di >= 0 ? ops[di].wS : nullptr; ib.wq2S = di >= 0 ? ops[ei].wS : nullptr; }
        }
        {
            const int kk = bq.k * bq.k, kkp = SGX_IRB_KKP(bq.k), rows = ((bq.outc + 31) / 32) * 32;
            std::vector<float> wp((size_t)rows * kkp, 0.f);
            for (int ch = 0; ch < bq.outc; ch++) { for (int t = 0; t < kk; t++) wp[(size_t)ch * kkp + t] = bq.hw[(size_t)ch * kk + t]; wp[(size_t)ch * kkp + kk] = bq.hb[ch]; }
            if ((rc = h->upload(&ib.wdp, wp))) return rc;
        }
        Op f; f.kind = OP_IRB; f.in0 = ai >= 0 ? ops[ai].in0 : bq.in0; f.out = m.out_blob; f.irb = ib; f.res_blob = m.res_blob;
        f.name = (ai >= 0 ? ops[ai].name + "+" : std::string()) + bq.name + "+" + c.name + (di >= 0 ? "+" + ops[di].name + "+" + ops[ei].name : std::string());
        f.inc = ib.Cin; f.outc = ib.Cout; f.H = bq.H; f.W = bq.W; f.Ho = bq.Ho; f.Wo = bq.Wo; f.k = bq.k; f.stride = bq.stride; f.hwc = c.hwc; f.hwc_off = c.hwc_off;
        const int ci = m.ci, last = di >= 0 ? ei : ci;
        if (ai >= 0) ops[ai].dead = true;
        bq.dead = true; if (last != ci) ops[ci].dead = true; if (di >= 0 && di != last) ops[di].dead = true;
        ops[last] = f;
    }
    return SGX_OK;
}

int Planner::fuse_se_gates()
{
    if (sw.irb != 1 || sw.legacy || !sw.se_gate) return SGX_OK;
    for (int di = 0; di < nops; di++) {
        Op &d = ops[di];
        if (d.dead || d.kind != OP_PW || d.hwc || d.in0 < 0) continue;
        const EpiClass cd = classify(d.epi);
        if (cd.mode != SGX_EMODE_ACT) continue;
        readers_all(d.out, R); if (R.size() != 1) continue;
        const int ei = R[0]; Op &e = ops[ei];
        if (e.kind != OP_PW || e.hwc || e.in0 != d.out || ei < di) continue;
        const EpiClass ce = classify(e.epi);
        if ((ce.mode != SGX_EMODE_GATE && ce.mode != SGX_EMODE_GATE_ADD) || ce.t0 != d.in0 || e.outc != d.inc || e.inc != d.outc) continue;
        if (!sgx_se_gate_supported(d.inc, d.outc) || h->is_output(d.out)) continue;
        SgxSeGate sg; memset(&sg, 0, sizeof sg);
        sg.Cout = d.inc; sg.Cq = d.outc; sg.HW = d.H * d.W;
        sg.se.bq1 = d.bias; sg.se.bq2 = e.bias; sg.se.qlo = cd.lo; sg.se.qhi = cd.hi; sg.se.gc1 = ce.c1; sg.se.glo = ce.lo; sg.se.ghi = ce.hi; sg.se.gc2 = ce.c2; sg.wq1 = d.wt; sg.wq2 = e.wt;
        const int rc = upload_se_interleaved(h, d, e, &sg.se.wq1p, &sg.se.wq2p); if (rc) return rc;
        Op f; f.kind = OP_SE_GATE; f.in0 = d.in0; f.out = e.out; f.sg = sg; f.res_blob = ce.mode == SGX_EMODE_GATE_ADD ? ce.t1 : -1;
        f.name = d.name + "+" + e.name; f.inc = d.inc; f.outc = e.outc; f.H = d.H; f.W = d.W; f.Ho = d.H; f.Wo = d.W;
        d.dead = true; ops[ei] = f;
    }
    return SGX_OK;
}

int Planner::merge_dual_heads()
{
    auto single_head = [](const Op &o) { return !o.dead && o.kind == OP_IRB && !o.irb.has_expand && o.irb.hwc && !o.irb.Cq && !o.irb.Cout2; };
    for (int i = 0; sw.irb_dual && i < nops; i++) {
        Op &a = ops[i];
        if (!single_head(a)) continue;
        for (int j = 0; j < nops; j++) {
            Op &b = ops[j];
            if (j == i || !single_head(b) || b.in0 != a.in0) continue;
            if (b.irb.K != a.irb.K || b.irb.S != a.irb.S || b.irb.Cexp != a.irb.Cexp || b.irb.H != a.irb.H || b.irb.W != a.irb.W || b.irb.act2 != a.irb.act2 ||
                b.irb.a2lo != a.irb.a2lo || b.irb.a2hi != a.irb.a2hi || b.irb.G != a.irb.G || b.irb.nbands != a.irb.nbands) continue;
            if (b.irb.Cout > 32 || b.irb.Cout > a.irb.Cout || b.irb.gemm != a.irb.gemm) continue;
            if (!sgx_irb_supported(a.irb.K, a.irb.S, (a.irb.Cout + 31) / 32, 0, false, a.irb.act2 == SGX_EMODE_HSWISH, 1)) continue;
            SgxIrb m = a.irb;
            m.Cout2 = b.irb.Cout; m.hwc_off2 = b.irb.hwc_off; m.ld2b = b.irb.ld2; m.wdp2 = b.irb.wdp; m.w2Tb = b.irb.w2T; m.b2b = b.irb.b2; m.w2Sb = b.irb.w2S;
            m.wd_b = b.irb.wd; m.bd_b = b.irb.bd; m.w2_b = b.irb.w2;
            if (sgx_irb_lds_bytes(m) > 160 * 1024) { m.nbuf = 1; if (sgx_irb_lds_bytes(m) > 160 * 1024) continue; }
            Op f = a; f.irb = m; f.irb_out2_blob = b.out; f.name = a.name + "|" + b.name;
            const int last = std::max(i, j);
            ops[i].dead = true; ops[j].dead = true; ops[last] = f; ops[last].dead = false;
            break;
        }
    }
    return SGX_OK;
}

int plan(sgx_det *h)
{
    if (!h->sw.fuse) return SGX_OK;
    Planner p(h); int rc;
    if ((rc = p.fuse_epilogues()) || (rc = p.fuse_blocks()) || (rc = p.fuse_irb()) || (rc = p.fuse_se_gates()) || (rc = p.merge_dual_heads())) return rc;
    std::vector<Op> live; for (const Op &o : h->ops) if (!o.dead) live.push_back(o);
    h->ops.swap(live);
    return SGX_OK;
}
}

static int launch_block_step(sgx_det *h, const Op &op, int batch, sgx_stream_t st, bool prepare)
{
    const Blob &A = h->blobs[op.in0]; const Blob &O = h->blobs[op.out];
    const float *res = op.res_blob >= 0 ? h->blobs[op.res_blob].d : nullptr; const size_t res_pitch = op.res_blob >= 0 ? h->blobs[op.res_blob].n : 0;
    switch (op.kind) {
    case OP_FUSED_BLOCK: {
        SgxFusedBlk fb = op.fb;
        fb.in = A.d; fb.in_pitch = A.n; fb.out = O.d; fb.out_pitch = O.n; fb.res = res; fb.res_pitch = res_pitch;
        if (fb.hrb) {
            SgxHrb q; memset(&q, 0, sizeof q);
            q.Cin = fb.Cin; q.Cmid = fb.Cmid; q.Cout = fb.Cout; q.Cq = fb.Cq; q.K = fb.K; q.S = fb.stride; q.pad = fb.pad; q.H = fb.H; q.W = fb.W; q.Ho = fb.Ho; q.Wo = fb.Wo;
            q.TOH = fb.TOH; q.TOW = fb.TOW; q.occ = fb.hrb_occ; q.tiles_x = fb.tiles_x; q.tiles_y = fb.tiles_y; q.lo1 = fb.lo1; q.hi1 = fb.hi1; q.lo2 = fb.lo2; q.hi2 = fb.hi2;
            q.in = fb.in; q.in_pitch = fb.in_pitch; q.out = fb.out; q.out_pitch = fb.out_pitch; q.res = fb.res; q.res_pitch = fb.res_pitch;
            q.w1S = (const sgx_q4 *)fb.w1S; q.ld1 = fb.ld1S; q.b1 = fb.b1; q.wd2 = fb.wd2; q.bd = fb.bd; q.w2S = (const sgx_q4 *)fb.w2S; q.ld2 = fb.ld2S; q.b2 = fb.b2;
            q.wq1S = (const sgx_q4 *)fb.wq1S; q.wq2S = (const sgx_q4 *)fb.wq2S; q.ldq1 = fb.ldq1S; q.ldq2 = fb.ldq2S; q.bq1 = fb.bq1; q.bq2 = fb.bq2;
            q.qlo = fb.qlo; q.qhi = fb.qhi; q.gc1 = fb.gc1; q.glo = fb.glo; q.ghi = fb.ghi; q.gc2 = fb.gc2;
            return sgx_hrb_dispatch(q, batch, st, prepare);
        }
        if (fb.v2) return sgx_fb2_dispatch(fb, batch, st, prepare);
#ifdef SGX_DEBUG_TAPS
        if (!prepare) SGX_LAUNCH_DYN(k_fused_block, dim3((unsigned)(fb.tiles_x * fb.tiles_y * batch)), dim3(256), sgx_fb_lds_floats(fb) * 4, st, fb);
        return SGX_OK;
#else
        return SGX_ERR_UNSUPPORTED;
#endif
    }
    case OP_SE_GATE: {
        SgxSeGate sg = op.sg;
        sg.y = A.d; sg.y_pitch = A.n; sg.out = O.d; sg.out_pitch = O.n; sg.res = res; sg.res_pitch = res_pitch;
        return sgx_se_gate_dispatch(sg, batch, st, prepare);
    }
    case OP_IRB: {
        SgxIrb ib = op.irb;
        ib.in = A.d; ib.in_pitch = A.n; ib.out = O.d; ib.out_pitch = O.n; ib.res = res; ib.res_pitch = res_pitch;
        if (op.irb_out2_blob >= 0) { ib.out2 = h->blobs[op.irb_out2_blob].d; ib.out2_pitch = h->blobs[op.irb_out2_blob].n; }
        return sgx_irb_dispatch(ib, batch, st, prepare);
    }
    default: return SGX_OK;
    }
}

static int finalise(sgx_det *h)
{
    const int B = h->max_batch, T = h->T;
    for (Op &o : h->ops) {
        std::vector<float>().swap(o.hw); std::vector<float>().swap(o.hb);
        Blob &ob = h->blobs[o.out]; if (!ob.d && ob.n) { if (h->alloc(&ob.d, ob.n * B)) return SGX_ERR_NOMEM; }
        if (o.irb_out2_blob >= 0) { Blob &o2 = h->blobs[o.irb_out2_blob]; if (!o2.d && o2.n) { if (h->alloc(&o2.d, o2.n * B)) return SGX_ERR_NOMEM; } }
    }
    {
        const int in_id = h->blob_id.at("input");
        int readers = 0; for (const Op &o : h->ops) readers += (o.in0 == in_id) + (o.in1 == in_id);
        if (h->sw.prefuse && h->sw.fuse && !h->sw.legacy && !h->ops.empty() && readers == 1 && stem2_ok(h, h->ops[0]) && h->ops[0].in0 == in_id) {
            Blob &ib = h->blobs[in_id];
            auto it = std::find(h->dev.begin(), h->dev.end(), (void *)ib.d);
            if (it != h->dev.end()) { (void)hipFree(ib.d); h->dev.erase(it); ib.d = nullptr; h->pre_fused = 1; }
        }
    }
    for (const Op &o : h->ops) { const int rc = launch_block_step(h, o, 1, nullptr, true); if (rc) return rc; }
    if ((size_t)h->num_priors * 4 != h->blobs[h->loc_blob].n || (size_t)h->num_priors * h->num_class != h->blobs[h->conf_blob].n) return SGX_ERR_INVALID;
    if (h->num_priors > SGX_DO_SORT || h->nms_top_k > SGX_DO_TOPK || (h->num_class - 1) * h->nms_top_k > SGX_DO_MERGE || h->num_class - 1 > 63 || h->num_class < 2 ||
        h->keep_top_k > SGX_DET_MAX) return SGX_ERR_UNSUPPORTED;
    int rc = h->upload(&h->d_priors, h->priors.data(), (size_t)h->num_priors * 4); if (rc) return rc;
    if (h->alloc(&h->d_cls_rows, (size_t)B * (h->num_class - 1) * SGX_DO_TOPK * 6) || h->alloc(&h->d_cls_count, (size_t)B * (h->num_class - 1)) || h->alloc(&h->d_results, (size_t)B)) return SGX_ERR_NOMEM;
    if (h->alloc(&h->d_cls_ncut, (size_t)B * (h->num_class - 1)) || h->alloc(&h->d_cls_next, (size_t)B * (h->num_class - 1)) || h->alloc(&h->d_cls_cont, (size_t)B * (h->num_class - 1)) || h->alloc(&h->d_sstar, (size_t)B)) return SGX_ERR_NOMEM;
#ifndef SGX_EMU
    SGX_CHECK_HIP(hipMemcpyToSymbol(HIP_SYMBOL(sgx_det_xcd_order), &h->sw.xcd, sizeof(int)));
#else
    sgx_det_xcd_order = h->sw.xcd;
#endif
    SGX_CHECK_HIP(hipMemset(h->d_results, 0, sizeof(sgx_det_result) * (size_t)B));
    std::vector<SgxDetTab> xt, yt; build_tab(h->W, T, xt); build_tab(h->H, T, yt);
    if ((rc = h->upload(&h->d_xt, xt)) || (rc = h->upload(&h->d_yt, yt))) return rc;
    return h->alloc(&h->d_img, (size_t)B * h->H * ((3 * h->W + 3) & ~3) + 4);
}

extern "C" int sgx_det_create(const char *param_text, const void *bin, size_t bin_bytes, int width, int height, int max_batch,
                              float detection_confidence_threshold, float dynamic_detection_confidence_threshold, sgx_det **out)
{
    if (!param_text || !bin || !out || width < 8 || height < 8 || width > SGX_PRE_MAXW || max_batch < 1) return SGX_ERR_INVALID;
    std::unique_ptr<sgx_det> h(new sgx_det());
    h->sw = det_switches();
    h->W = width; h->H = height; h->max_batch = max_batch; h->det_th = detection_confidence_threshold; h->dyn_th = dynamic_detection_confidence_threshold;
    int rc = parse_param(param_text, h->layers);
    if (rc != SGX_OK) return rc;
    Loader load{ h.get(), (const uint8_t *)bin, bin_bytes };
    if ((rc = load.run()) || (rc = plan(h.get())) || (rc = finalise(h.get()))) return rc;
    *out = h.release();
    return SGX_OK;
}

static SgxEpi make_epi(const sgx_det *h, const Op &op, size_t tpitch)
{
    SgxEpi e; memset(&e, 0, sizeof e);
    e.tpitch = tpitch;
    for (const EpiStep &st : op.epi) {
        SgxEpiStep &d = e.s[e.n++];
        d.op = st.op; d.src = st.src; d.a = st.a; d.b = st.b; d.t = st.tensor >= 0 ? h->blobs[st.tensor].d : nullptr;
    }
    const EpiClass k = classify_epi(e.s, (size_t)e.n);
    e.mode = k.mode;
    if (k.mode == SGX_EMODE_ACT || k.mode == SGX_EMODE_HSWISH || k.mode == SGX_EMODE_GATE || k.mode == SGX_EMODE_GATE_ADD) { e.lo = k.lo; e.hi = k.hi; }
    if (k.mode == SGX_EMODE_HSWISH || k.mode == SGX_EMODE_GATE || k.mode == SGX_EMODE_GATE_ADD) { e.c1 = k.c1; e.c2 = k.c2; }
    if (k.i0 >= 0) e.t0 = e.s[k.i0].t;
    if (k.i1 >= 0) e.t1 = e.s[k.i1].t;
    return e;
}

#ifdef SGX_EMU
static void sgx_pw3_emu(int inc, int outc, int N, int batch, const float *in, size_t in_pitch, const unsigned short *wS, int ldw, const float *bias, float *out, size_t out_pitch,
                        const SgxEpi &epi, int hwc, int hwc_off)
{
    const int nks = (inc + 15) / 16;
    auto split = [](float x, float *t) {
        const unsigned short h0 = sgx_bf16_rne(x); t[0] = sgx_bf16_to_f32(h0); const float r1 = x - t[0];
        const unsigned short h1 = sgx_bf16_rne(r1); t[1] = sgx_bf16_to_f32(h1); t[2] = sgx_bf16_to_f32(sgx_bf16_rne(r1 - t[1]));
    };
    std::vector<float> xs((size_t)nks * 16 * 3);
    for (int b = 0; b < batch; b++) for (int n = 0; n < N; n++) {
        const float *X = in + (size_t)b * in_pitch;
        for (int k = 0; k < nks * 16; k++) split(X[(size_t)std::min(k, inc - 1) * N + n], &xs[(size_t)k * 3]);
        for (int o = 0; o < outc; o++) {
            float acc = bias[o];
            for (int s = 0; s < nks; s++) {
                static const int TA[6] = { 0, 1, 2, 0, 1, 0 }, TB[6] = { 2, 1, 0, 1, 0, 0 };
                for (int q = 0; q < 6; q++) {
                    double sum = 0;
                    for (int kk = 0; kk < 16; kk++) {
                        const int hf = kk >> 3, j = kk & 7;
                        const float a = sgx_bf16_to_f32(wS[((((size_t)s * 3 + TA[q]) * 2 + hf) * ldw + o) * 8 + j]);
                        sum += (double)a * (double)xs[(size_t)(16 * s + kk) * 3 + TB[q]];
                    }
                    acc = (float)((double)acc + sum);
                }
            }
            const float v = sgx_epi(epi, acc, (size_t)b * epi.tpitch + (size_t)o * N + n);
            float *Y = out + (size_t)b * out_pitch;
            if (hwc) Y[(size_t)hwc_off + (size_t)n * outc + o] = v; else Y[(size_t)o * N + n] = v;
        }
    }
}
#endif

static bool pw_bf16x3(const sgx_det *h, const Op &op) { return op.kind == OP_PW && h->sw.gemm == 1 && op.wS && op.inc >= h->sw.pw3_mink; }

struct PwTile { int ocb, pxb, nxt, noc, grid; };
static PwTile pw_tile(const int (*cand)[3], int ncand, int sub, int total, int force = 0)
{
    PwTile t = { 1, 1, 0, 0, 0 }; long best_score = -1;
    for (int c = 0; c < ncand; c++) {
        const int cb = cand[c][0], cp = cand[c][1];
        const long nwg = (long)((total + 128 * cp - 1) / (128 * cp)) * ((sub + cb - 1) / cb);
        const int padded = ((sub + cb - 1) / cb) * cb;
        const long fill = std::min(nwg, 512L);
        const long score = fill * 1000000L + (long)(1000 - (padded - sub) * 100) * 100L + cand[c][2];
        if (score > best_score) { best_score = score; t.ocb = cb; t.pxb = cp; }
    }
    if (force) { t.ocb = force / 10; t.pxb = force % 10; }
    t.nxt = (total + 128 * t.pxb - 1) / (128 * t.pxb); t.noc = (sub + t.ocb - 1) / t.ocb;
    t.grid = ((t.nxt + 7) / 8) * 8 * t.noc;
    return t;
}
static const int pw2_cand[7][3] = { {4, 2, 8}, {3, 2, 6}, {2, 2, 4}, {1, 4, 4}, {2, 1, 2}, {1, 2, 2}, {1, 1, 1} };
static const int pw3_cand[8][3] = { {2, 2, 42}, {4, 1, 81}, {3, 1, 61}, {5, 1, 101}, {1, 4, 24}, {2, 1, 41}, {1, 2, 22}, {1, 1, 21} };

struct DwBands { int nplanes, P, RB, nbands, ngroups, rows; };
static DwBands dw_bands(const Op &op, int batch, int pitch, int budget)
{
    DwBands g; g.nplanes = batch * op.outc; g.P = 1; g.RB = op.Ho;
    const int rin_full = (op.Ho - 1) * op.stride + op.k;
    if (rin_full * pitch <= budget) g.P = std::max(1, std::min(std::min(budget / (rin_full * pitch), 16), g.nplanes / 2048));
    else {
        const int rbmax = std::max(1, (budget / pitch - op.k) / op.stride + 1);
        int nb = (op.Ho + rbmax - 1) / rbmax;
        nb = std::max(nb, std::min((2048 + g.nplanes - 1) / g.nplanes, std::max(1, op.Ho / 4)));
        g.RB = (op.Ho + nb - 1) / nb;
    }
    g.nbands = (op.Ho + g.RB - 1) / g.RB; g.ngroups = (g.nplanes + g.P - 1) / g.P; g.rows = (g.RB - 1) * op.stride + op.k;
    return g;
}

static int run_op(sgx_det *h, const Op &op, int batch, sgx_stream_t st)
{
    const Blob &A = h->blobs[op.in0]; const Blob &O = h->blobs[op.out];
    const DetSwitches &sw = h->sw;
    switch (op.kind) {
    case OP_PW: {
        const int N = op.H * op.W;
        const size_t big = (size_t)batch * std::max(std::max(A.n, O.n), (size_t)op.outc * N) * 4;
        const SgxEpi e = make_epi(h, op, (size_t)op.outc * N);
        if (h->sw.legacy || !op.wtT || (op.inc & 1) || big >= 0xFFFFFFFFull) {
            SGX_LAUNCH(k_conv_pw, dim3((N + 63) / 64, (op.outc + 63) / 64, batch), dim3(256), st, op.inc, op.outc, N, A.d, A.n, op.wt, op.bias, O.d, O.n, e, op.hwc, op.hwc_off);
            break;
        }
        const int sub = (op.outc + 31) / 32, total = batch * N;
        if (pw_bf16x3(h, op)) {
#ifdef SGX_EMU
            sgx_pw3_emu(op.inc, op.outc, N, batch, A.d, A.n, (const unsigned short *)op.wS, op.ldw, op.bias, O.d, O.n, e, op.hwc, op.hwc_off);
#else
            const PwTile t = pw_tile(pw3_cand, 8, sub, total, sw.pw3_force);
#define SGX_PW3(OCB_, PXB_) do { auto kfn = k_conv_pw3<OCB_, PXB_>; SGX_LAUNCH(kfn, dim3(t.grid), dim3(256), st, op.inc, op.outc, N, total, A.d, A.n, (const sgx_u32x4 *)op.wS, op.bias, \
                                                                               O.d, O.n, e, op.hwc, op.hwc_off, t.nxt, t.noc, op.ldw, 1); } while (0)
            switch (t.ocb * 10 + t.pxb) {
            case 22: SGX_PW3(2, 2); break; case 41: SGX_PW3(4, 1); break; case 31: SGX_PW3(3, 1); break; case 51: SGX_PW3(5, 1); break; case 14: SGX_PW3(1, 4); break;
            case 21: SGX_PW3(2, 1); break; case 12: SGX_PW3(1, 2); break; default: SGX_PW3(1, 1); break;
            }
#undef SGX_PW3
#endif
            break;
        }
        const PwTile t = pw_tile(pw2_cand, 7, sub, total);
#define SGX_PW2(OCB_, PXB_) do { auto kfn = k_conv_pw2<OCB_, PXB_>; SGX_LAUNCH(kfn, dim3(t.grid), dim3(256), st, op.inc, op.outc, N, total, A.d, A.n, op.wtT, op.bias, \
                                                                               O.d, O.n, e, op.hwc, op.hwc_off, t.nxt, t.noc, op.ldw, sw.pw2_direct); } while (0)
        switch (t.ocb * 10 + t.pxb) {
        case 42: SGX_PW2(4, 2); break; case 32: SGX_PW2(3, 2); break; case 22: SGX_PW2(2, 2); break; case 14: SGX_PW2(1, 4); break;
        case 21: SGX_PW2(2, 1); break; case 12: SGX_PW2(1, 2); break; default: SGX_PW2(1, 1); break;
        }
#undef SGX_PW2
        break; }
    case OP_FUSED_BLOCK: case OP_SE_GATE: case OP_IRB: return launch_block_step(h, op, batch, st, false);
    case OP_KXK: {
        const SgxEpi e = make_epi(h, op, (size_t)op.outc * op.Ho * op.Wo);
        const int budget = sw.dw_budget;
        const int Wp = (op.Wo - 1) * op.stride + op.k;
        const int nbx4 = (op.Wo + 3) / 4, pitch4 = ((nbx4 - 1) * 4 * op.stride + 3 * op.stride + op.k + 3) & ~3;
#ifdef SGX_DEBUG_TAPS
        if (sw.dw3 && !h->sw.legacy && op.depthwise && op.wtP) {
            SgxDw3 d; int px = 1; size_t lds3 = 0;
            if (sgx_dw3_plan(op.outc, op.H, op.W, op.Ho, op.Wo, op.k, op.stride, op.pad, e.mode, &d, &px, &lds3)) {
                d.in = A.d; d.in_pitch = A.n; d.wd2 = op.wtP; d.bias = op.bias; d.out = O.d; d.out_pitch = O.n; d.epi = e;
                sgx_dw3_launch(d, op.k, op.stride, px, lds3, batch, st);
                break;
            }
        }
#endif
        if (sw.dw2 && !h->sw.legacy && op.depthwise && (op.k == 3 || op.k == 5) && (op.stride == 1 || op.stride == 2) && pitch4 * op.k <= budget) {
            const DwBands g = dw_bands(op, batch, pitch4, budget);
            const int KW = (op.k * op.k + 1 + 3) & ~3;
            const size_t lds = ((size_t)g.P * g.rows * pitch4 + (size_t)g.P * KW) * 4;
#define SGX_DW2(K_, S_) do { auto kfn = k_conv_dw2<K_, S_>; SGX_LAUNCH_DYN(kfn, dim3(g.ngroups * g.nbands), dim3(256), lds, st, op.outc, op.H, op.W, op.Ho, op.Wo, op.pad, g.P, g.RB, g.nbands, g.nplanes, pitch4, \
                                                                          sgx_magic(std::min(g.RB, op.Ho) * nbx4), sgx_magic(nbx4), A.d, op.wt, op.bias, O.d, e); } while (0)
            if (op.k == 3 && op.stride == 1) SGX_DW2(3, 1); else if (op.k == 3) SGX_DW2(3, 2); else if (op.stride == 1) SGX_DW2(5, 1); else SGX_DW2(5, 2);
#undef SGX_DW2
        } else if (!h->sw.legacy && op.depthwise && (op.k == 3 || op.k == 5) && Wp * op.k <= budget) {
            const DwBands g = dw_bands(op, batch, Wp, budget);
            const size_t lds = ((size_t)g.P * g.rows * Wp + (size_t)g.P * (op.k * op.k + 1)) * 4;
#define SGX_DW(K_) do { auto kfn = k_conv_dw<K_>; SGX_LAUNCH_DYN(kfn, dim3(g.ngroups * g.nbands), dim3(256), lds, st, op.outc, op.H, op.W, op.Ho, op.Wo, op.stride, op.pad, g.P, g.RB, g.nbands, g.nplanes, \
                                                                sgx_magic(((std::min(g.RB, op.Ho) - 1) * op.stride + op.k) * Wp), sgx_magic(Wp), sgx_magic(op.Wo), A.d, op.wt, op.bias, O.d, e); } while (0)
            if (op.k == 3) SGX_DW(3); else SGX_DW(5);
#undef SGX_DW
        } else if (stem2_ok(h, op)) {
            const Stem2Geom g = stem2_geom(h, op);
            auto kfn = k_conv_stem2<3>;
            SGX_LAUNCH_DYN(kfn, dim3(g.nbands, batch), dim3(256), g.lds, st, op.outc, op.H, op.W, op.Ho, op.Wo, op.pad, g.RB, g.pitch4, sgx_magic(g.nbx4), A.d, A.n, op.wtT, op.bias, O.d, O.n, e);
        } else if (!h->sw.legacy && !op.depthwise && op.wtT && op.outc <= 16 && op.inc * Wp * op.k <= budget) {
            const int RB = std::min(op.Ho, std::max(1, (budget / (op.inc * Wp) - op.k) / op.stride + 1)), nbands = (op.Ho + RB - 1) / RB;
            const size_t lds = (size_t)op.inc * ((RB - 1) * op.stride + op.k) * Wp * 4;
            SGX_LAUNCH_DYN(k_conv_stem, dim3(nbands, batch), dim3(256), lds, st, op.inc, op.outc, op.H, op.W, op.Ho, op.Wo, op.k, op.stride, op.pad, RB, sgx_magic(((RB - 1) * op.stride + op.k) * Wp), sgx_magic(Wp), sgx_magic(op.Wo),
                           A.d, A.n, op.wtT, op.bias, O.d, O.n, e);
        } else
            SGX_LAUNCH(k_conv_kxk, dim3((op.Ho * op.Wo + 255) / 256, op.outc, batch), dim3(256), st, op.inc, op.outc, op.H, op.W, op.Ho, op.Wo, op.k, op.stride, op.pad, op.depthwise,
                       A.d, A.n, op.wt, op.bias, O.d, O.n, e);
        break; }
    case OP_BINARY: {
        const Blob &Bb = h->blobs[op.in1];
        const size_t n = A.n * batch; const int g = (int)std::min<size_t>((n + 255) / 256, 8192);
        SGX_LAUNCH(k_binary, dim3(g), dim3(256), st, n, op.bop, A.d, Bb.scalar ? A.d : Bb.d, Bb.scalar ? 1 : 0, Bb.sval, O.d);
        break; }
    case OP_UNARY: { const size_t n = A.n * batch; const int g = (int)std::min<size_t>((n + 255) / 256, 8192); SGX_LAUNCH(k_unary, dim3(g), dim3(256), st, n, op.act, op.lo, op.hi, A.d, O.d); break; }
    case OP_PERMUTE_INTO: SGX_LAUNCH(k_permute_hwc_into, dim3((op.C * op.rows + 255) / 256, batch), dim3(256), st, op.C, op.rows, A.d, A.n, O.d, O.n, op.off); break;
    case OP_COPY_INTO: SGX_LAUNCH(k_copy_into, dim3(((int)A.n + 255) / 256, batch), dim3(256), st, (int)A.n, A.d, A.n, O.d, O.n, op.off); break;
    case OP_SOFTMAX: SGX_LAUNCH(k_softmax_rows, dim3((op.rows + 255) / 256, batch), dim3(256), st, op.rows, op.C, A.d, A.n, O.d, O.n); break;
    }
    return SGX_OK;
}

static int run_first_step(sgx_det *h, const uint8_t *d_img, int pitch, int batch, sgx_stream_t st)
{
    const int T = h->T;
    if (!h->pre_fused) {
        SGX_LAUNCH(k_det_preprocess, dim3(T, batch), dim3(256), st, batch, d_img, h->W, h->H, pitch, h->d_xt, h->d_yt, T, 123.675f, 116.28f, 103.53f, h->blobs[h->blob_id.at("input")].d);
        return SGX_OK;
    }
    const Op &op = h->ops[0]; const Blob &O = h->blobs[op.out];
    const SgxEpi e = make_epi(h, op, (size_t)op.outc * op.Ho * op.Wo);
    const Stem2Geom g = stem2_geom(h, op);
    SGX_LAUNCH_DYN(k_stem_pre, dim3(g.nbands * batch), dim3(256), g.lds + (size_t)(T + (g.RB - 1) * 2 + 3) * sizeof(SgxDetTab), st, d_img, h->H, pitch, h->d_xt, h->d_yt, T, 123.675f, 116.28f, 103.53f, g.nbands, batch,
                   op.outc, op.Ho, op.Wo, op.pad, g.RB, g.pitch4, sgx_magic(g.pitch4), sgx_magic(g.nbx4), op.wtT, op.bias, O.d, O.n, e);
    return SGX_OK;
}

#ifndef SGX_EMU
static int abandon_capture(sgx_stream_t st, int rc) { hipGraph_t g = nullptr; (void)hipStreamEndCapture(st, &g); if (g) (void)hipGraphDestroy(g); return rc; }
static int capture_forked(sgx_det *h, size_t first, int batch, sgx_stream_t st, int lanes, hipGraph_t *graph)
{
    const int n = (int)h->ops.size();
    auto root = [&](int b) { return b >= 0 ? h->resolve(b) : b; };
    std::vector<std::vector<int>> rd(n), wr(n); std::vector<char> partial(n, 0);
    for (int i = (int)first; i < n; i++) {
        const Op &o = h->ops[i];
        for (int b : { o.in0, o.in1, o.res_blob }) if (b >= 0 && !h->blobs[b].scalar) rd[i].push_back(root(b));
        for (const EpiStep &e : o.epi) if (e.tensor >= 0) rd[i].push_back(root(e.tensor));
        wr[i].push_back(root(o.out)); if (o.irb_out2_blob >= 0) wr[i].push_back(root(o.irb_out2_blob));
        partial[i] = (o.hwc || o.kind == OP_PERMUTE_INTO || o.kind == OP_COPY_INTO || (o.kind == OP_IRB && o.irb.hwc)) ? 1 : 0;
    }
    auto hits = [](const std::vector<int> &a, const std::vector<int> &b) { for (int x : a) for (int y : b) if (x == y) return true; return false; };
    std::vector<std::vector<int>> deps(n), users(n);
    for (int i = (int)first; i < n; i++)
        for (int j = (int)first; j < i; j++)
            if (hits(wr[j], rd[i]) || hits(rd[j], wr[i]) || (hits(wr[j], wr[i]) && !(partial[i] && partial[j]))) { deps[i].push_back(j); users[j].push_back(i); }
    std::vector<int> prio(n, 1), heir(n, -1);
    for (int i = n - 1; i >= (int)first; i--)
        for (int u : users[i]) if (prio[u] + 1 > prio[i]) { prio[i] = prio[u] + 1; heir[i] = u; }
    lanes = std::max(1, std::min(lanes, 8));
    while ((int)h->fork_streams.size() < lanes - 1) { hipStream_t q; SGX_CHECK_HIP(hipStreamCreateWithFlags(&q, hipStreamNonBlocking)); h->fork_streams.push_back(q); }
    std::vector<hipStream_t> L(lanes); L[0] = st; for (int l = 1; l < lanes; l++) L[l] = h->fork_streams[l - 1];
    std::vector<int> tail(lanes, -1), lane_of(n, 0); std::vector<char> started(lanes, 0); started[0] = 1;
    std::vector<hipEvent_t> done(n, nullptr);
    std::vector<hipEvent_t> pool((size_t)n + 2 * lanes); size_t next_ev = 0;
    for (hipEvent_t &e : pool) { SGX_CHECK_HIP(hipEventCreateWithFlags(&e, hipEventDisableTiming)); h->fork_events.push_back(e); }
    SGX_CHECK_HIP(hipStreamBeginCapture(st, hipStreamCaptureModeThreadLocal));
#define CAP_CHECK(x) do { if ((x) != hipSuccess) return abandon_capture(st, SGX_ERR_DEVICE); } while (0)
    for (int i = (int)first; i < n; i++) {
        int lane = -1;
        for (int j : deps[i]) if (tail[lane_of[j]] == j && heir[j] == i) { lane = lane_of[j]; break; }
        if (lane < 0 && !deps[i].empty()) {
            for (int l = 1; l < lanes && lane < 0; l++) {
                const int t = tail[l];
                if (t < 0 || heir[t] < 0 || heir[t] < i) lane = l;
            }
            if (lane < 0) for (int j : deps[i]) if (tail[lane_of[j]] == j) { lane = lane_of[j]; break; }
        }
        if (lane < 0) lane = 0;
        for (int j : deps[i]) if (lane_of[j] != lane) { CAP_CHECK(hipStreamWaitEvent(L[lane], done[j], 0)); started[lane] = 1; }
        if (!started[lane]) {
            hipEvent_t e = pool[next_ev++];
            CAP_CHECK(hipEventRecord(e, L[0])); CAP_CHECK(hipStreamWaitEvent(L[lane], e, 0)); started[lane] = 1;
        }
        { const int rc = run_op(h, h->ops[i], batch, L[lane]); if (rc != SGX_OK) return abandon_capture(st, rc); }
        lane_of[i] = lane; tail[lane] = i;
        if (!users[i].empty()) {
            hipEvent_t e = pool[next_ev++]; CAP_CHECK(hipEventRecord(e, L[lane])); done[i] = e;
        }
    }
    for (int l = 1; l < lanes; l++) if (started[l] && tail[l] >= 0) {
        hipEvent_t e = pool[next_ev++];
        CAP_CHECK(hipEventRecord(e, L[l])); CAP_CHECK(hipStreamWaitEvent(L[0], e, 0));
    }
#undef CAP_CHECK
    SGX_CHECK_HIP(hipStreamEndCapture(st, graph));
    return SGX_OK;
}
#endif

extern "C" int sgx_det_forward_batch_dev(sgx_det *h, const uint8_t *d_img, int pitch, int batch, const float **d_loc, const float **d_conf, void *stream_)
{
    if (!h || !d_img || batch < 1 || batch > h->max_batch || pitch < ((3 * h->W + 3) & ~3) || (pitch & 3) || ((uintptr_t)d_img & 3)) return SGX_ERR_INVALID;
    sgx_stream_t st = (sgx_stream_t)stream_;
    sgx_prof_begin(SGX_K_DET_FWD, st);
    int rc = run_first_step(h, d_img, pitch, batch, st);
    if (rc != SGX_OK) return rc;
    const size_t first = h->pre_fused ? 1 : 0;
#ifndef SGX_EMU
    if (st != nullptr && !h->sw.no_graph) {
        auto it = h->graphs.find(batch);
        if (it == h->graphs.end()) {
            hipGraph_t graph = nullptr; hipGraphExec_t exec = nullptr;
            if (h->sw.fork_lanes > 1) { if ((rc = capture_forked(h, first, batch, st, h->sw.fork_lanes, &graph)) != SGX_OK) return rc; }
            else {
                SGX_CHECK_HIP(hipStreamBeginCapture(st, hipStreamCaptureModeThreadLocal));
                for (size_t i = first; i < h->ops.size(); i++) if ((rc = run_op(h, h->ops[i], batch, st)) != SGX_OK) return abandon_capture(st, rc);
                SGX_CHECK_HIP(hipStreamEndCapture(st, &graph));
            }
            std::vector<hipGraphExec_t> execs;
            for (int e = 0; e < std::max(1, std::min(h->sw.graph_execs, 4)); e++) { SGX_CHECK_HIP(hipGraphInstantiate(&exec, graph, nullptr, nullptr, 0)); execs.push_back(exec); }
            (void)hipGraphDestroy(graph);
            it = h->graphs.emplace(batch, execs).first;
        }
        { unsigned &turn = h->graph_turn[batch]; SGX_CHECK_HIP(hipGraphLaunch(it->second[turn % it->second.size()], st)); turn++; }
    } else
#endif
    for (size_t i = first; i < h->ops.size(); i++) if ((rc = run_op(h, h->ops[i], batch, st)) != SGX_OK) return rc;
    sgx_prof_end(SGX_K_DET_FWD, st);
    SGX_CHECK_HIP(hipGetLastError());
    if (d_loc) *d_loc = h->blobs[h->loc_blob].d;
    if (d_conf) *d_conf = h->blobs[h->conf_blob].d;
    return SGX_OK;
}

SGX_TAP int sgx_det_debug_time_ops(sgx_det *h, const uint8_t *d_img, int pitch, int batch, int reps, float *ms, int cap, int *nops)
{
    if (!h || !d_img || !ms || !nops || batch < 1 || batch > h->max_batch || reps < 1) return SGX_ERR_INVALID;
    const int skip = h->pre_fused;
    *nops = (int)h->ops.size() + 1 - skip;
    if (cap < *nops) return SGX_ERR_INVALID;
#ifndef SGX_EMU
    hipEvent_t a, b; SGX_CHECK_HIP(hipEventCreate(&a)); SGX_CHECK_HIP(hipEventCreate(&b));
    for (int i = 0; i < *nops; i++) {
        float tot = 0.f;
        for (int r = 0; r < reps + 1; r++) {
            SGX_CHECK_HIP(hipEventRecord(a, 0));
            const int rc = i == 0 ? run_first_step(h, d_img, pitch, batch, 0) : run_op(h, h->ops[i - 1 + skip], batch, 0);
            if (rc != SGX_OK) { (void)hipEventDestroy(a); (void)hipEventDestroy(b); return rc; }
            SGX_CHECK_HIP(hipEventRecord(b, 0)); SGX_CHECK_HIP(hipEventSynchronize(b));
            float t = 0.f; SGX_CHECK_HIP(hipEventElapsedTime(&t, a, b)); if (r) tot += t;
        }
        ms[i] = tot / reps;
    }
    (void)hipEventDestroy(a); (void)hipEventDestroy(b);
    return SGX_OK;
#else
    return SGX_ERR_UNSUPPORTED;
#endif
}

SGX_TAP int sgx_det_debug_run_step(sgx_det *h, const uint8_t *d_img, int pitch, int batch, int i, int reps, void *stream)
{
    if (!h || !d_img || batch < 1 || batch > h->max_batch || reps < 1) return SGX_ERR_INVALID;
    const int skip = h->pre_fused, nops = (int)h->ops.size() + 1 - skip;
    if (i < 0 || i >= nops) return SGX_ERR_INVALID;
    for (int r = 0; r < reps; r++) { const int rc = i == 0 ? run_first_step(h, d_img, pitch, batch, (sgx_stream_t)stream) : run_op(h, h->ops[i - 1 + skip], batch, (sgx_stream_t)stream); if (rc != SGX_OK) return rc; }
    return SGX_OK;
}

extern "C" int sgx_det_plan_step(const sgx_det *h, int i, char *buf, int cap)
{
    if (!h || !buf || cap < 16 || i < 0 || i > (int)h->ops.size() - h->pre_fused) return SGX_ERR_INVALID;
    if (i == 0 && !h->pre_fused) { snprintf(buf, cap, "preprocess %dx%d->%d", h->W, h->H, h->T); return SGX_OK; }
    if (i == 0) { const Op &s0 = h->ops[0]; snprintf(buf, cap, "kxk %s c%d->%d k%d s%d %dx%d->%dx%d epi%d pre %dx%d->%d", s0.name.c_str(), s0.inc, s0.outc, s0.k, s0.stride, s0.H, s0.W, s0.Ho, s0.Wo,
                                                     (int)s0.epi.size() + (s0.act ? 1 : 0), h->W, h->H, h->T); return SGX_OK; }
    const Op &o = h->ops[i - 1 + h->pre_fused];
    static const char *kn[] = { "pw", "kxk", "binary", "unary", "permute_into", "copy_into", "softmax", "block", "irb", "se_gate" };
    if (o.kind == OP_SE_GATE) { snprintf(buf, cap, "se_gate %s c%d->%d->%d %dx%d%s", o.name.c_str(), o.sg.Cout, o.sg.Cq, o.sg.Cout, o.H, o.W, o.res_blob >= 0 ? " +res" : ""); return SGX_OK; }
    if (o.kind == OP_PW || o.kind == OP_KXK)
        snprintf(buf, cap, "%s %s c%d->%d k%d s%d %s%dx%d->%dx%d epi%d%s%s", kn[o.kind], o.name.c_str(), o.inc, o.outc, o.k, o.stride, o.depthwise ? "dw " : "", o.H, o.W,
                 o.kind == OP_PW ? o.H : o.Ho, o.kind == OP_PW ? o.W : o.Wo, (int)o.epi.size() + (o.act ? 1 : 0), o.hwc ? " hwc" : "", pw_bf16x3(h, o) ? " bf16x3" : "");
    else if (o.kind == OP_FUSED_BLOCK)
        snprintf(buf, cap, "block %s c%d->%d->%d k%d s%d %dx%d->%dx%d tile %dx%d%s%s%s", o.name.c_str(), o.fb.Cin, o.fb.Cmid, o.fb.Cout, o.fb.K, o.fb.stride, o.H, o.W, o.Ho, o.Wo, o.fb.TOH, o.fb.TOW,
                 o.fb.Cq ? " se" : "", o.res_blob >= 0 ? " +res" : "", o.fb.hrb ? (o.fb.hrb_occ == 4 ? " hrb4 bf16x3" : o.fb.hrb_occ == 3 ? " hrb3 bf16x3" : " hrb2 bf16x3") : "");
    else if (o.kind == OP_IRB)
        snprintf(buf, cap, "irb %s c%d->%d->%d q%d k%d s%d %dx%d->%dx%d G%d bands%d buf%d%s%s%s%s", o.name.c_str(), o.irb.Cin, o.irb.Cexp, o.irb.Cout, o.irb.Cq, o.irb.K, o.irb.S, o.H, o.W, o.Ho, o.Wo,
                 o.irb.G, o.irb.nbands, o.irb.nbuf, o.irb.has_expand ? "" : " noexp", o.res_blob >= 0 ? " +res" : "", o.hwc ? (o.irb.Cout2 ? " hwc dual" : " hwc") : "", o.irb.gemm == 1 ? " bf16x3" : "");
    else snprintf(buf, cap, "%s %s n=%zu", kn[o.kind], o.name.c_str(), h->blobs[o.in0].n);
    return SGX_OK;
}

extern "C" int sgx_det_info(const sgx_det *h, int32_t *num_priors, int32_t *num_class, int32_t *num_kernels, double *gmac)
{
    if (!h) return SGX_ERR_INVALID;
    if (num_priors) *num_priors = h->num_priors; if (num_class) *num_class = h->num_class; if (num_kernels) *num_kernels = (int)h->ops.size() + 1 - h->pre_fused; if (gmac) *gmac = h->gmac;
    return SGX_OK;
}

SGX_TAP int sgx_det_debug_read_blob(sgx_det *h, const char *name, int image, float *dst, int cap, int *n)
{
    if (!h || !name || !n) return SGX_ERR_INVALID;
    auto it = h->blob_id.find(name); if (it == h->blob_id.end()) return SGX_ERR_INVALID;
    const int id = h->resolve(it->second);
    const Blob &b = h->blobs[id];
    if (!b.d || image < 0 || image >= h->max_batch) return SGX_ERR_INVALID;
    *n = (int)b.n;
    if (dst && cap >= (int)b.n) SGX_CHECK_HIP(hipMemcpy(dst, b.d + (size_t)image * b.n, b.n * 4, hipMemcpyDeviceToHost));
    return SGX_OK;
}

static int run_detection_output(sgx_det *h, int batch, sgx_det_result *d_results, float *d_boxes, int32_t *d_nboxes, int max_boxes, int32_t *d_have_dynamic, sgx_stream_t st);

extern "C" int sgx_det_detect_batch_dev(sgx_det *h, const uint8_t *d_img, int pitch, int batch, sgx_det_result *d_results,
                                        float *d_boxes, int32_t *d_nboxes, int max_boxes, int32_t *d_have_dynamic, void *stream_)
{
    if (!h || !d_results || ((d_boxes != nullptr) != (d_nboxes != nullptr)) || (d_boxes && max_boxes < 1)) return SGX_ERR_INVALID;
    const float *dl = nullptr, *dc = nullptr;
    int rc = sgx_det_forward_batch_dev(h, d_img, pitch, batch, &dl, &dc, stream_);
    if (rc != SGX_OK) return rc;
    return run_detection_output(h, batch, d_results, d_boxes, d_nboxes, max_boxes, d_have_dynamic, (sgx_stream_t)stream_);
}

static int run_detection_output(sgx_det *h, int batch, sgx_det_result *d_results, float *d_boxes, int32_t *d_nboxes, int max_boxes, int32_t *d_have_dynamic, sgx_stream_t st)
{
    SgxDetOut P; P.n = h->num_priors; P.nc = h->num_class; P.nms_top_k = h->nms_top_k; P.keep_top_k = h->keep_top_k; P.nms_th = h->nms_th; P.conf_th = h->conf_th;
    P.var0 = h->dvar[0]; P.var1 = h->dvar[1]; P.var2 = h->dvar[2]; P.var3 = h->dvar[3];
    if (h->sw.skip_output) return SGX_OK;
    sgx_prof_begin(SGX_K_DET_OUT, st);
    const dim3 grid(h->num_class - 1, batch);
    const size_t lds_full = (size_t)std::max(h->num_priors, 7 * SGX_DO_TOPK) * 4 + 16, lds_first = (size_t)std::max(h->num_priors, 7 * (SGX_DO_FIRST + 1)) * 4 + 16;
    const float *loc = h->blobs[h->loc_blob].d, *conf = h->blobs[h->conf_blob].d;
    const int *no_cont = nullptr; const uint32_t *no_sstar = nullptr; int *no_ncut = nullptr; uint32_t *no_next = nullptr;
    if (h->sw.out_single) {
        SGX_LAUNCH_DYN(k_det_class_nms<0>, grid, dim3(256), lds_full, st, P, loc, conf, h->d_priors, h->d_cls_rows, h->d_cls_count, no_ncut, no_next, no_cont, no_sstar);
    } else {
        SGX_LAUNCH_DYN(k_det_class_nms<SGX_DO_FIRST>, grid, dim3(256), lds_first, st, P, loc, conf, h->d_priors, h->d_cls_rows, h->d_cls_count, h->d_cls_ncut, h->d_cls_next, no_cont, no_sstar);
        SGX_LAUNCH(k_det_cut, dim3(batch), dim3(256), st, P, h->d_cls_rows, h->d_cls_count, h->d_cls_ncut, h->d_cls_next, h->d_sstar, h->d_cls_cont);
        SGX_LAUNCH_DYN(k_det_class_nms<0>, grid, dim3(256), lds_full, st, P, loc, conf, h->d_priors, h->d_cls_rows, h->d_cls_count, no_ncut, no_next, h->d_cls_cont, h->d_sstar);
    }
    h->last_out_batch = h->sw.out_single ? 0 : batch;
    SGX_LAUNCH(k_det_merge, dim3(batch), dim3(256), st, P, h->d_cls_rows, h->d_cls_count, h->det_th, h->dyn_th, h->W, h->H, h->T, d_results, d_boxes, d_nboxes, max_boxes, d_have_dynamic);
    sgx_prof_end(SGX_K_DET_OUT, st);
    SGX_CHECK_HIP(hipGetLastError());
    return SGX_OK;
}

SGX_TAP int sgx_det_debug_detection_output(sgx_det *h, const float *loc, const float *conf, int batch, sgx_det_result *results)
{
    if (!h || !loc || !conf || !results || batch < 1 || batch > h->max_batch) return SGX_ERR_INVALID;
    SGX_CHECK_HIP(hipMemcpy(h->blobs[h->loc_blob].d, loc, sizeof(float) * 4 * (size_t)h->num_priors * batch, hipMemcpyHostToDevice));
    SGX_CHECK_HIP(hipMemcpy(h->blobs[h->conf_blob].d, conf, sizeof(float) * (size_t)h->num_priors * h->num_class * batch, hipMemcpyHostToDevice));
    int rc = run_detection_output(h, batch, h->d_results, nullptr, nullptr, 0, nullptr, (sgx_stream_t)0);
    if (rc != SGX_OK) return rc;
    SGX_CHECK_HIP(hipMemcpy(results, h->d_results, sizeof(sgx_det_result) * batch, hipMemcpyDeviceToHost));
    return SGX_OK;
}

SGX_TAP int sgx_det_debug_continued(sgx_det *h, int *count)
{
    if (!h || !count) return SGX_ERR_INVALID;
    std::vector<int> cont((size_t)h->last_out_batch * (h->num_class - 1));
    if (!cont.empty()) SGX_CHECK_HIP(hipMemcpy(cont.data(), h->d_cls_cont, cont.size() * sizeof(int), hipMemcpyDeviceToHost));
    *count = 0; for (int v : cont) *count += v;
    return SGX_OK;
}

extern "C" int sgx_det_detect(sgx_det *h, const uint8_t *images, int pitch, int batch, sgx_det_result *results)
{
    if (!h || !images || !results || batch < 1 || batch > h->max_batch || pitch < 3 * h->W) return SGX_ERR_INVALID;
    const int ipitch = (3 * h->W + 3) & ~3;
    for (int b = 0; b < batch; b++)
        for (int y = 0; y < h->H; y++)
            SGX_CHECK_HIP(hipMemcpyAsync(h->d_img + ((size_t)b * h->H + y) * ipitch, images + ((size_t)b * h->H + y) * pitch, (size_t)3 * h->W, hipMemcpyHostToDevice, 0));
    int rc = sgx_det_detect_batch_dev(h, h->d_img, ipitch, batch, h->d_results, nullptr, nullptr, 0, nullptr, nullptr);
    if (rc != SGX_OK) return rc;
    SGX_CHECK_HIP(hipMemcpy(results, h->d_results, sizeof(sgx_det_result) * batch, hipMemcpyDeviceToHost));
    return SGX_OK;
}

extern "C" int sgx_dynamic_mask_batch_dev(int batch, int cap, const sgx_keypoint *d_keys, const int32_t *d_n, const float *d_prev_xy, const double *d_F,
                                          const float *d_boxes, const int32_t *d_nboxes, int max_boxes, uint8_t *d_keep, void *stream)
{
    if (batch < 1 || cap < 1 || !d_keys || !d_n || !d_prev_xy || !d_F || !d_boxes || !d_nboxes || !d_keep || max_boxes < 0) return SGX_ERR_INVALID;
    sgx_prof_begin(SGX_K_MASK, (sgx_stream_t)stream);
    SGX_LAUNCH(k_dynamic_mask, dim3((cap + 255) / 256, batch), dim3(256), (sgx_stream_t)stream, cap, (const uint8_t *)d_keys, d_n, d_prev_xy, d_F, d_boxes, d_nboxes, max_boxes, d_keep);
    sgx_prof_end(SGX_K_MASK, (sgx_stream_t)stream);
    SGX_CHECK_HIP(hipGetLastError());
    return SGX_OK;
}

extern "C" int sgx_frame_compact_keys_batch_dev(int batch, int cap, const sgx_keypoint *d_keys, const uint8_t *d_desc, const int32_t *d_n, const uint8_t *d_keep,
                                                const int32_t *d_have_dynamic, int nfeatures, sgx_keypoint *d_keys_out, uint8_t *d_desc_out, int32_t *d_n_out, void *stream)
{
    if (batch < 1 || cap < 1 || !d_keys || !d_desc || !d_n || !d_keep || !d_keys_out || !d_desc_out || !d_n_out || (const void *)d_keys == (const void *)d_keys_out) return SGX_ERR_INVALID;
    sgx_prof_begin(SGX_K_MASK, (sgx_stream_t)stream);
    SGX_LAUNCH(k_compact_keys, dim3(batch), dim3(256), (sgx_stream_t)stream, cap, (const uint8_t *)d_keys, d_desc, d_n, d_keep, d_have_dynamic, (float)nfeatures * 0.1f,
               (uint8_t *)d_keys_out, d_desc_out, d_n_out);
    sgx_prof_end(SGX_K_MASK, (sgx_stream_t)stream);
    SGX_CHECK_HIP(hipGetLastError());
    return SGX_OK;
}
```

### sg_slam_amd/csrc/sgx_lanes.h

```cpp
#pragma once
#include "sgx_rt.h"
#include "sgx_det_block.h"
#include "sgx_det_bf16.h"

#ifndef SGX_EMU
typedef float vf; typedef int vi; typedef unsigned vu; typedef bool vb;
typedef sgx_f2 vf2;
typedef sgx_f32x16 vf16;
typedef sgx_u32x4 vu4;
typedef sgx_u32x4 sgx_q4;
struct VB3 { vu4 t0, t1, t2; };
#define SGX_WAVES_BEGIN(w) { const int w = SGX_UNIFORM((int)threadIdx.x >> 6);
#define SGX_WAVES_END }
#define SGX_WAVE_EXIT() return
#define SGX_WPRIV_DECL(type, name, count) type name[count]
#define SGX_WPRIV_BIND(name, w) ((void)0)
SGX_DEV vi v_lane() { return (int)threadIdx.x & 63; }
SGX_DEV vf v_sel(vb c, vf a, vf b) { return c ? a : b; }
SGX_DEV vi v_seli(vb c, vi a, vi b) { return c ? a : b; }
SGX_DEV vi v_min(vi a, vi b) { return a < b ? a : b; }
SGX_DEV vu v_u(vi a) { return (unsigned)a; }
SGX_DEV vf v_fma(vf a, vf b, vf c) { return fmaf(a, b, c); }
SGX_DEV vf v_clip(vf v, float lo, float hi) { return __builtin_amdgcn_fmed3f(v, lo, hi); }
SGX_DEV vf v_clipv(vf v, float lo, vf hi) { return __builtin_amdgcn_fmed3f(v, lo, hi); }
SGX_DEV vf v_ld(const float *base, vu byte_off) { return *(const float *)((const char *)base + byte_off); }
SGX_DEV void v_st(float *base, vu byte_off, vf v, vb m) { if (m) *(float *)((char *)base + byte_off) = v; }
SGX_DEV vu4 v_ldq(const sgx_q4 *base, vi idx) { return base[idx]; }
SGX_DEV vf2 v_lds_ld2(const sgx_f2 *E, vi idx) { return E[idx]; }
SGX_DEV void v_lds_st2(sgx_f2 *E, vi idx, vf x, vf y, vb m) { if (m) E[idx] = sgx_mk2(x, y); }
SGX_DEV vu4 v_lds_ldq(const sgx_q4 *E, vi idx) { return E[idx]; }
SGX_DEV void v_lds_stq(sgx_q4 *E, vi idx, vu4 v, vb m) { if (m) E[idx] = v; }
SGX_DEV vf v_lds_ld(const float *E, vi idx) { return E[idx]; }
SGX_DEV void v_lds_st(float *E, vi idx, vf v) { E[idx] = v; }
SGX_DEV vf2 v_mk2(vf x, vf y) { return sgx_mk2(x, y); }
SGX_DEV vf v_x(vf2 a) { return a.x; }
SGX_DEV vf v_y(vf2 a) { return a.y; }
SGX_DEV vf2 v_fma2_w(sgx_f2 w, vf2 b, vf2 c) { return sgx_fma2_w(w, b, c); }
SGX_DEV VB3 v_split3x8(const vf (&v)[8]) { const SgxB3 s = sgx_split3x8(v); VB3 r; r.t0 = s.t0; r.t1 = s.t1; r.t2 = s.t2; return r; }
SGX_DEV vf16 v_mfma3(const vu4 &a0, const vu4 &a1, const vu4 &a2, const VB3 &b, vf16 acc)
{
    acc = SGX_MFMA_BF16(a0, b.t2, acc); acc = SGX_MFMA_BF16(a1, b.t1, acc); acc = SGX_MFMA_BF16(a2, b.t0, acc);
    acc = SGX_MFMA_BF16(a0, b.t1, acc); acc = SGX_MFMA_BF16(a1, b.t0, acc);
    return SGX_MFMA_BF16(a0, b.t0, acc);
}
SGX_DEV void v_swap32(vf x, vf y, vf &nx, vf &ny)
{
    const auto r = __builtin_amdgcn_permlane32_swap(__float_as_uint(x), __float_as_uint(y), false, false);
    nx = __uint_as_float(r[0]); ny = __uint_as_float(r[1]);
}
#else
template <class T> struct sgx_lv {
    T v[64];
    sgx_lv() { for (int l = 0; l < 64; l++) v[l] = T(); }
    sgx_lv(T s) { for (int l = 0; l < 64; l++) v[l] = s; }
};
typedef sgx_lv<float> vf; typedef sgx_lv<int> vi; typedef sgx_lv<unsigned> vu; typedef sgx_lv<bool> vb;
#define SGX_LV_BIN(op, R)                                                                                                                                   \
    template <class T> static inline sgx_lv<R> operator op(const sgx_lv<T> &a, const sgx_lv<T> &b) { sgx_lv<R> r; for (int l = 0; l < 64; l++) r.v[l] = (R)(a.v[l] op b.v[l]); return r; } \
    template <class T> static inline sgx_lv<R> operator op(const sgx_lv<T> &a, T b) { sgx_lv<R> r; for (int l = 0; l < 64; l++) r.v[l] = (R)(a.v[l] op b); return r; }                  \
    template <class T> static inline sgx_lv<R> operator op(T a, const sgx_lv<T> &b) { sgx_lv<R> r; for (int l = 0; l < 64; l++) r.v[l] = (R)(a op b.v[l]); return r; }
#define SGX_LV_ARITH(op) SGX_LV_BIN(op, T)
SGX_LV_ARITH(+) SGX_LV_ARITH(-) SGX_LV_ARITH(*) SGX_LV_ARITH(/) SGX_LV_ARITH(&) SGX_LV_ARITH(|) SGX_LV_ARITH(>>) SGX_LV_ARITH(<<)
SGX_LV_BIN(<, bool) SGX_LV_BIN(<=, bool) SGX_LV_BIN(>, bool) SGX_LV_BIN(>=, bool) SGX_LV_BIN(==, bool) SGX_LV_BIN(!=, bool)
static inline vb operator!(const vb &a) { vb r; for (int l = 0; l < 64; l++) r.v[l] = !a.v[l]; return r; }
struct vf2 { vf x, y; };
struct vf16 { vf r[16]; vf &operator[](int i) { return r[i]; } const vf &operator[](int i) const { return r[i]; } };
struct vu4 { vu c[4]; vu &operator[](int i) { return c[i]; } const vu &operator[](int i) const { return c[i]; } };
struct sgx_q4 { unsigned v[4]; };
struct VB3 { vu4 t0, t1, t2; };
#define SGX_WAVES_BEGIN(w) for (int w = 0; w < (int)blockDim.x / 64; ++w) {
#define SGX_WAVES_END }
#define SGX_WAVE_EXIT() continue
#define SGX_WPRIV_DECL(type, name, count) static thread_local type name##_store[16][count]
#define SGX_WPRIV_BIND(name, w) auto *name = name##_store[w]
static inline vi v_lane() { vi r; for (int l = 0; l < 64; l++) r.v[l] = l; return r; }
static inline vf v_sel(const vb &c, const vf &a, const vf &b) { vf r; for (int l = 0; l < 64; l++) r.v[l] = c.v[l] ? a.v[l] : b.v[l]; return r; }
static inline vi v_seli(const vb &c, const vi &a, const vi &b) { vi r; for (int l = 0; l < 64; l++) r.v[l] = c.v[l] ? a.v[l] : b.v[l]; return r; }
static inline vi v_min(const vi &a, const vi &b) { vi r; for (int l = 0; l < 64; l++) r.v[l] = a.v[l] < b.v[l] ? a.v[l] : b.v[l]; return r; }
static inline vu v_u(const vi &a) { vu r; for (int l = 0; l < 64; l++) r.v[l] = (unsigned)a.v[l]; return r; }
static inline vf v_fma(const vf &a, const vf &b, const vf &c) { vf r; for (int l = 0; l < 64; l++) r.v[l] = fmaf(a.v[l], b.v[l], c.v[l]); return r; }
static inline vf v_clip(const vf &v, float lo, float hi) { vf r; for (int l = 0; l < 64; l++) r.v[l] = fminf(fmaxf(v.v[l], lo), hi); return r; }
static inline vf v_clipv(const vf &v, float lo, const vf &hi) { vf r; for (int l = 0; l < 64; l++) r.v[l] = fminf(fmaxf(v.v[l], lo), hi.v[l]); return r; }
static inline vf v_ld(const float *base, const vu &off) { vf r; for (int l = 0; l < 64; l++) r.v[l] = *(const float *)((const char *)base + off.v[l]); return r; }
static inline void v_st(float *base, const vu &off, const vf &v, const vb &m) { for (int l = 0; l < 64; l++) if (m.v[l]) *(float *)((char *)base + off.v[l]) = v.v[l]; }
static inline vu4 v_ldq(const sgx_q4 *base, const vi &idx) { vu4 r; for (int l = 0; l < 64; l++) for (int j = 0; j < 4; j++) r.c[j].v[l] = base[idx.v[l]].v[j]; return r; }
static inline vf2 v_lds_ld2(const sgx_f2 *E, const vi &idx) { vf2 r; for (int l = 0; l < 64; l++) { r.x.v[l] = E[idx.v[l]].x; r.y.v[l] = E[idx.v[l]].y; } return r; }
static inline void v_lds_st2(sgx_f2 *E, const vi &idx, const vf &x, const vf &y, const vb &m) { for (int l = 0; l < 64; l++) if (m.v[l]) { E[idx.v[l]].x = x.v[l]; E[idx.v[l]].y = y.v[l]; } }
static inline vu4 v_lds_ldq(const sgx_q4 *E, const vi &idx) { return v_ldq(E, idx); }
static inline void v_lds_stq(sgx_q4 *E, const vi &idx, const vu4 &v, const vb &m) { for (int l = 0; l < 64; l++) if (m.v[l]) for (int j = 0; j < 4; j++) E[idx.v[l]].v[j] = v.c[j].v[l]; }
static inline vf v_lds_ld(const float *E, const vi &idx) { vf r; for (int l = 0; l < 64; l++) r.v[l] = E[idx.v[l]]; return r; }
static inline void v_lds_st(float *E, const vi &idx, const vf &v) { for (int l = 0; l < 64; l++) E[idx.v[l]] = v.v[l]; }
static inline vf2 v_mk2(const vf &x, const vf &y) { vf2 r; r.x = x; r.y = y; return r; }
static inline vf v_x(const vf2 &a) { return a.x; }
static inline vf v_y(const vf2 &a) { return a.y; }
static inline vf2 v_fma2_w(sgx_f2 w, const vf2 &b, const vf2 &c) { vf2 r; for (int l = 0; l < 64; l++) { r.x.v[l] = fmaf(w.x, b.x.v[l], c.x.v[l]); r.y.v[l] = fmaf(w.y, b.y.v[l], c.y.v[l]); } return r; }
static inline VB3 v_split3x8(const vf (&v)[8])
{
    VB3 b;
    for (int l = 0; l < 64; l++) for (int j = 0; j < 8; j++) {
        const float x = v[j].v[l];
        const unsigned short h0 = sgx_bf16_rne(x); const float r1 = x - sgx_bf16_to_f32(h0);
        const unsigned short h1 = sgx_bf16_rne(r1); const unsigned short h2 = sgx_bf16_rne(r1 - sgx_bf16_to_f32(h1));
        const int sh = 16 * (j & 1); const unsigned keep = ~(0xffffu << sh);
        b.t0.c[j >> 1].v[l] = (b.t0.c[j >> 1].v[l] & keep) | ((unsigned)h0 << sh);
        b.t1.c[j >> 1].v[l] = (b.t1.c[j >> 1].v[l] & keep) | ((unsigned)h1 << sh);
        b.t2.c[j >> 1].v[l] = (b.t2.c[j >> 1].v[l] & keep) | ((unsigned)h2 << sh);
    }
    return b;
}
static inline float sgx_lv_bf16(const vu4 &a, int lane, int j) { return sgx_bf16_to_f32((unsigned short)(a.c[j >> 1].v[lane] >> (16 * (j & 1)))); }
static inline vf16 v_mfma1(const vu4 &a, const vu4 &b, const vf16 &c)
{
    vf16 d;
    for (int half = 0; half < 2; half++) for (int i = 0; i < 32; i++) for (int r = 0; r < 16; r++) {
        const int row = (r & 3) + 8 * (r >> 2) + 4 * half;
        double sum = 0;
        for (int k = 0; k < 16; k++) sum += (double)sgx_lv_bf16(a, 32 * (k >> 3) + row, k & 7) * (double)sgx_lv_bf16(b, 32 * (k >> 3) + i, k & 7);
        d.r[r].v[32 * half + i] = (float)((double)c.r[r].v[32 * half + i] + sum);
    }
    return d;
}
static inline vf16 v_mfma3(const vu4 &a0, const vu4 &a1, const vu4 &a2, const VB3 &b, vf16 acc)
{
    acc = v_mfma1(a0, b.t2, acc); acc = v_mfma1(a1, b.t1, acc); acc = v_mfma1(a2, b.t0, acc);
    acc = v_mfma1(a0, b.t1, acc); acc = v_mfma1(a1, b.t0, acc);
    return v_mfma1(a0, b.t0, acc);
}
static inline void v_swap32(const vf &x, const vf &y, vf &nx, vf &ny)
{
    vf a, b;
    for (int l = 0; l < 32; l++) { a.v[l] = x.v[l]; a.v[32 + l] = y.v[l]; b.v[l] = x.v[32 + l]; b.v[32 + l] = y.v[32 + l]; }
    nx = a; ny = b;
}
#endif
```

### sg_slam_amd/detector.py

```python
import ctypes as C
import numpy as np
from .capi import DetResult, _vp
from ._lib import load

CLASS_NAMES = ["background", "aeroplane", "bicycle", "bird", "boat", "bottle", "bus", "car", "cat", "chair", "cow", "diningtable",
               "dog", "horse", "motorbike", "person", "pottedplant", "sheep", "sofa", "train", "tvmonitor"]


class Detector2D:
    def __init__(self, detection_confidence_threshold, dynamic_detection_confidence_threshold, param_path=None, bin_path=None,
                 param_text=None, bin_bytes=None, width=640, height=480, max_batch=1, lib=None, fuse=True, legacy_kernels=False, block_fusion=False, irb=None, gemm=None):
        self.lib = lib if lib is not None else load()
        if param_text is None:
            param_text = open(param_path or './Thirdparty/ncnn_model/mobilenetv3_ssdlite_voc.param').read()
        if bin_bytes is None:
            bin_bytes = open(bin_path or './Thirdparty/ncnn_model/mobilenetv3_ssdlite_voc.bin', 'rb').read()
        self._bin = bin_bytes
        h = C.c_void_p()
        taps = dict(fusion=1 if fuse else 0, legacy_kernels=1 if legacy_kernels else 0, block_fusion=1 if block_fusion else 0,
                    irb=-1 if irb is None else (2 if irb is True else int(irb)), gemm=-1 if gemm is None else (0 if gemm in (0, 'f32') else 1))
        default = dict(fusion=1, legacy_kernels=0, block_fusion=0, irb=-1, gemm=-1)
        if taps != default or self.lib.has_taps:
            for k, v in taps.items(): self.lib.tap('sgx_det_debug_set_' + k)(v)
        self.lib.check(self.lib.dll.sgx_det_create(param_text.encode(), bin_bytes, len(bin_bytes), width, height, max_batch,
                                                   float(detection_confidence_threshold), float(dynamic_detection_confidence_threshold), C.byref(h)), 'sgx_det_create')
        if self.lib.has_taps:
            for k, v in default.items(): self.lib.tap('sgx_det_debug_set_' + k)(v)
        self.h = h; self.width, self.height, self.max_batch = width, height, max_batch
        npri, ncls, nk = C.c_int32(), C.c_int32(), C.c_int32(); g = C.c_double()
        self.lib.check(self.lib.dll.sgx_det_info(self.h, C.byref(npri), C.byref(ncls), C.byref(nk), C.byref(g)))
        self.num_priors, self.num_class, self.num_kernels, self.gmac = npri.value, ncls.value, nk.value, g.value
        self.gemm = 'bf16x3' if self.lib.dll.sgx_det_gemm_mode(self.h) == 1 else 'f32'
        self.mvObjects2D = []; self.mbHaveDynamicObjectForMapping = False; self.mbHaveDynamicObjectForRmDynamicFeature = False
        self.mvPotentialDynamicBorderForMapping = []; self.mvPotentialDynamicBorderForRmDynamicFeature = []

    def close(self):
        if getattr(self, 'h', None):
            self.lib.dll.sgx_det_destroy(self.h); self.h = None

    def __del__(self):
        try: self.close()
        except Exception: pass

    def detect_batch(self, images):
        imgs = np.ascontiguousarray(images, np.uint8)
        if imgs.ndim == 3: imgs = imgs[None]
        B = imgs.shape[0]
        res = (DetResult * B)()
        self.lib.check(self.lib.dll.sgx_det_detect(self.h, _vp(imgs), imgs.shape[2] * 3, B, res), 'sgx_det_detect')
        return res

    def detect_batch_dev(self, d_img, pitch, batch, d_results, d_boxes=None, d_nboxes=None, max_boxes=0, d_have_dynamic=None, stream=None):
        self.lib.check(self.lib.dll.sgx_det_detect_batch_dev(self.h, _vp(d_img), pitch, batch, _vp(d_results), None if d_boxes is None else _vp(d_boxes),
                                                             None if d_nboxes is None else _vp(d_nboxes), max_boxes, None if d_have_dynamic is None else _vp(d_have_dynamic),
                                                             None if stream is None else C.c_void_p(stream)), 'sgx_det_detect_batch_dev')

    def detect(self, bgr):
        r = self.detect_batch(bgr)[0]
        rect = lambda o: (o.x, o.y, o.w, o.h)
        self.raw = np.array([[d.label, d.score, d.xmin, d.ymin, d.xmax, d.ymax] for d in r.raw[:r.n_raw]], np.float32).reshape(-1, 6)
        self.mvObjects2D = [(o.id, CLASS_NAMES[o.id], o.prob, rect(o)) for o in r.objects[:r.n_objects]]
        self.mbHaveDynamicObjectForMapping = bool(r.have_dynamic_for_mapping)
        self.mbHaveDynamicObjectForRmDynamicFeature = bool(r.have_dynamic_for_rm_feature)
        self.mvPotentialDynamicBorderForMapping = [rect(o) for o in r.map_boxes[:r.n_map_boxes]]
        self.mvPotentialDynamicBorderForRmDynamicFeature = [rect(o) for o in r.rm_boxes[:r.n_rm_boxes]]

    def has_blob(self, name):
        n = C.c_int(0)
        return self.lib.tap('sgx_det_debug_read_blob')(self.h, name.encode(), 0, None, 0, C.byref(n)) == 0

    def time_ops(self, d_img, batch, reps=5):
        ms = np.zeros(self.num_kernels, 'f4'); n = C.c_int(0)
        self.lib.check(self.lib.tap('sgx_det_debug_time_ops')(self.h, _vp(d_img), self.width * 3, batch, reps, _vp(ms), len(ms), C.byref(n)))
        out = []
        for i in range(n.value):
            buf = C.create_string_buffer(256); self.lib.check(self.lib.dll.sgx_det_plan_step(self.h, i, buf, 256)); out.append((buf.value.decode(), float(ms[i])))
        return out

    def op_descriptions(self):
        out = []
        for i in range(self.num_kernels):
            buf = C.create_string_buffer(256)
            if self.lib.dll.sgx_det_plan_step(self.h, i, buf, 256) != 0: break
            out.append(buf.value.decode())
        return out

    def debug_blob(self, name, image=0):
        n = C.c_int(0)
        self.lib.check(self.lib.tap('sgx_det_debug_read_blob')(self.h, name.encode(), image, None, 0, C.byref(n)))
        out = np.zeros(n.value, 'f4')
        self.lib.check(self.lib.tap('sgx_det_debug_read_blob')(self.h, name.encode(), image, _vp(out), n.value, C.byref(n)))
        return out
```

Measured before the change: 29390.

## Fuse detector tail layers into single LDS-resident megakernel

Adds a fused kernel that runs the last chain of small spatial layers of the detector (depthwise 3x3 stride-2, bf16x3 pointwise convs and the classification/location heads) inside one workgroup per 1-2 frames. Intermediates stay in up to 160KB of LDS, with buffer offsets chosen by a liveness-based allocator. The aim is to remove the many tiny kernel launches and global-memory round trips those late layers cost. The head uses fp32 MFMA, and the whole tail runs with few workgroups, so parallelism is low. It is on by default, can be switched off with an environment variable, and comes with debug timing taps.

```diff
diff --git a/include/sgx_debug.h b/include/sgx_debug.h
--- a/include/sgx_debug.h
+++ b/include/sgx_debug.h
@@ -29,6 +29,8 @@
 int sgx_det_debug_set_gemm(int mode);
 int sgx_det_debug_set_legacy_kernels(int on);
 int sgx_det_debug_time_ops(sgx_det *h, const uint8_t *d_img, int pitch, int batch, int reps, float *ms, int cap, int *nops);
+int sgx_det_debug_tail_steps(const sgx_det *h, int *steps, int cap, int *n);
+int sgx_det_debug_time_tail(sgx_det *h, int batch, int reps, float *ms);
 int sgx_det_debug_run_step(sgx_det *h, const uint8_t *d_img, int pitch, int batch, int step, int reps, void *stream);
 int sgx_orb_debug_run_octree(sgx_orb *h, int level, const uint32_t *packed, int n, uint32_t *out_sel, int cap, int *nsel);
 
diff --git a/sg_slam_amd/capi.py b/sg_slam_amd/capi.py
--- a/sg_slam_amd/capi.py
+++ b/sg_slam_amd/capi.py
@@ -86,7 +86,7 @@
     'sgx_orb_debug_level_geometry', 'sgx_orb_debug_set_unfused_pyramid', 'sgx_orb_debug_read_level', 'sgx_orb_debug_read_candidates',
     'sgx_orb_debug_run_octree', 'sgx_pose_opt_debug_set_threads', 'sgx_ba_debug_set_solver', 'sgx_ba_debug_set_jobs', 'sgx_ba_debug_set_init', 'sgx_ba_debug_last_plan', 'sgx_det_debug_read_blob',
     'sgx_det_debug_detection_output', 'sgx_det_debug_continued', 'sgx_debug_flow_affine_batch_dev', 'sgx_det_debug_set_fusion', 'sgx_det_debug_set_legacy_kernels',
-    'sgx_det_debug_set_block_fusion', 'sgx_det_debug_set_irb', 'sgx_det_debug_set_gemm', 'sgx_det_debug_time_ops', 'sgx_det_debug_run_step', 'sgx_flow_debug_read_level',
+    'sgx_det_debug_set_block_fusion', 'sgx_det_debug_set_irb', 'sgx_det_debug_set_gemm', 'sgx_det_debug_time_ops', 'sgx_det_debug_run_step', 'sgx_det_debug_tail_steps', 'sgx_det_debug_time_tail', 'sgx_flow_debug_read_level',
     'sgx_flow_debug_level_size', 'sgx_debug_corun_bf16', 'sgx_pnp_debug_betas',
 ]
 
@@ -241,6 +241,8 @@
                 getattr(d, 'sgx_det_debug_set_' + nm).argtypes = [C.c_int]
             d.sgx_det_debug_time_ops.argtypes = [vp, vp, C.c_int, C.c_int, C.c_int, vp, C.c_int, C.POINTER(C.c_int)]
             d.sgx_det_debug_run_step.argtypes = [vp, vp, C.c_int, C.c_int, C.c_int, C.c_int, vp]
+            d.sgx_det_debug_tail_steps.argtypes = [vp, vp, C.c_int, C.POINTER(C.c_int)]
+            d.sgx_det_debug_time_tail.argtypes = [vp, C.c_int, C.c_int, C.POINTER(C.c_float)]
             d.sgx_debug_flow_affine_batch_dev.argtypes = [C.c_int, C.c_int, vp, vp, vp, vp, vp, C.c_int, vp, vp]
             d.sgx_flow_debug_read_level.argtypes = [vp, C.c_int, C.c_int, C.c_int, vp]
             d.sgx_debug_corun_bf16.argtypes = [C.c_int, C.c_int, C.c_int, vp]
diff --git a/sg_slam_amd/csrc/sgx_det.cpp b/sg_slam_amd/csrc/sgx_det.cpp
--- a/sg_slam_amd/csrc/sgx_det.cpp
+++ b/sg_slam_amd/csrc/sgx_det.cpp
@@ -3,6 +3,7 @@
 #include "sgx_det_irb.h"
 #include "sgx_det_bf16.h"
 #include "sgx_det_hrb.h"
+#include "sgx_det_tail.h"
 #include "sgx_prof.h"
 #include "../../include/sgx.h"
 #ifdef SGX_DEBUG_TAPS
@@ -68,6 +69,7 @@
     int stem_words = 13824, dw2 = 1, dw3 = 0, dw_budget = 8192, pw3_mink = 64, pw3_force = 0, pw2_direct = 1;
     int no_graph = 0, fork_lanes = SGX_DET_FORK_LANES, graph_execs = SGX_DET_GRAPH_EXECS, skip_output = 0;
     int out_single = 0;
+    int tail = 1;
 };
 
 struct sgx_det {
@@ -88,6 +90,7 @@
     int *d_cls_ncut = nullptr, *d_cls_cont = nullptr; uint32_t *d_cls_next = nullptr, *d_sstar = nullptr;
     int last_out_batch = 0;
     double gmac = 0;
+    std::vector<int> tail_ops; std::vector<char> tail_member; int tail_first = -1; SgxTail tail; size_t tail_lds = 0;
 #ifndef SGX_EMU
     std::map<int, std::vector<hipGraphExec_t>> graphs;
     std::map<int, unsigned> graph_turn;
@@ -139,6 +142,7 @@
     s.no_graph = sgx_getenv("SGX_DET_NO_GRAPH") != nullptr; env("SGX_DET_FORK", s.fork_lanes); env("SGX_DET_EXECS", s.graph_execs);
     s.skip_output = sgx_getenv("SGX_DET_SKIP_OUTPUT") != nullptr;
     s.out_single = sgx_getenv("SGX_DET_OUT_SINGLE") != nullptr;
+    env("SGX_DET_TAIL", s.tail);
     return s;
 }
 
@@ -154,6 +158,7 @@
     return g;
 }
 static SgxEpi make_epi(const sgx_det *h, const Op &op, size_t tpitch);
+static int group_tail(sgx_det *h);
 static bool stem2_ok(const sgx_det *h, const Op &op)
 {
     if (op.kind != OP_KXK || !h->sw.dw2 || h->sw.legacy || op.depthwise || !op.wtT || op.outc > 16 || op.inc != 3 || op.k != 3 || op.stride != 2) return false;
@@ -820,6 +825,7 @@
         }
     }
     for (const Op &o : h->ops) { const int rc = launch_block_step(h, o, 1, nullptr, true); if (rc) return rc; }
+    { const int rc = group_tail(h); if (rc) return rc; }
     if ((size_t)h->num_priors * 4 != h->blobs[h->loc_blob].n || (size_t)h->num_priors * h->num_class != h->blobs[h->conf_blob].n) return SGX_ERR_INVALID;
     if (h->num_priors > SGX_DO_SORT || h->nms_top_k > SGX_DO_TOPK || (h->num_class - 1) * h->nms_top_k > SGX_DO_MERGE || h->num_class - 1 > 63 || h->num_class < 2 ||
         h->keep_top_k > SGX_DET_MAX) return SGX_ERR_UNSUPPORTED;
@@ -1037,6 +1043,115 @@
     return SGX_OK;
 }
 
+
+static bool tail_dw_ok(const Op &o)
+{
+    return o.kind == OP_KXK && o.depthwise && o.inc == o.outc && sgx_tail_dw_ok(o.outc, o.k, o.stride, o.pad) && !o.hwc && classify(o.epi).mode == SGX_EMODE_ACT;
+}
+static bool tail_pw_ok(const sgx_det *h, const Op &o, int F)
+{
+    return o.kind == OP_PW && !o.hwc && o.wtT && pw_bf16x3(h, o) && classify(o.epi).mode == SGX_EMODE_ACT && sgx_tail_pw3_ok(o.inc, o.outc, F * o.H * o.W);
+}
+static bool tail_head_ok(const Op &o, int F)
+{
+    const SgxIrb &ib = o.irb;
+    return o.kind == OP_IRB && !ib.has_expand && ib.hwc && !ib.Cq && ib.gemm == 0 && !ib.has_res && ib.K == 3 && ib.S == 1 && ib.pad == 1 && ib.act2 == SGX_EMODE_ACT && ib.nbands == 1 &&
+           ib.Cin == ib.Cexp && sgx_tail_head_ok(ib.Cexp, ib.Cout, ib.Cout2, F * ib.H * ib.W, SGX_TAIL_THREADS / 64);
+}
+static int group_tail(sgx_det *h)
+{
+    const int n = (int)h->ops.size();
+    h->tail_ops.clear(); h->tail_member.assign(n, 0); h->tail_first = -1;
+    if (!h->sw.tail || !h->sw.fuse || h->sw.legacy || h->sw.gemm != 1 || h->sw.irb != 1) return SGX_OK;
+    for (int F = 2; F >= 1 && h->tail_ops.empty(); F--) {
+        for (int i0 = (int)h->pre_fused; i0 < n && h->tail_ops.empty(); i0++) {
+            if (!tail_dw_ok(h->ops[i0]) || F * h->ops[i0].Ho * h->ops[i0].Wo > 64) continue;
+            std::vector<int> chain{ i0 };
+            for (int cur = h->ops[i0].out;;) {
+                int next = -1, cnt = 0;
+                for (int j = chain.back() + 1; j < n; j++) {
+                    const Op &o = h->ops[j];
+                    if (o.in0 == cur && (tail_dw_ok(o) || tail_pw_ok(h, o, F))) { if (next < 0) next = j; cnt++; }
+                }
+                if (cnt != 1) break;
+                chain.push_back(next); cur = h->ops[next].out;
+            }
+            while (!chain.empty() && h->ops[chain.back()].kind != OP_PW) chain.pop_back();
+            if (chain.size() < 3) continue;
+            SgxTail T; memset(&T, 0, sizeof T); T.F = F;
+            std::vector<int> members, src_layer;
+            std::map<int, int> layer_of_blob;
+            bool ok = true;
+            for (int ci : chain) {
+                const Op &o = h->ops[ci];
+                auto it = layer_of_blob.find(o.in0);
+                if (ci != i0 && it == layer_of_blob.end()) { ok = false; break; }
+                src_layer.push_back(ci == i0 ? -1 : it->second); layer_of_blob[o.out] = (int)members.size(); members.push_back(ci);
+                for (int j = 0; j < n; j++) if (h->ops[j].in0 == o.out && j > ci && tail_head_ok(h->ops[j], F)) { src_layer.push_back(layer_of_blob[o.out]); members.push_back(j); }
+            }
+            if (!ok || (int)members.size() > SGX_TAIL_MAXL) continue;
+            T.nl = (int)members.size();
+            struct Buf { int off, size, end; };
+            std::vector<Buf> bufs(T.nl); int top = 0;
+            for (int li = 0; li < T.nl; li++) {
+                const Op &o = h->ops[members[li]];
+                const bool head = o.kind == OP_IRB;
+                Buf b; b.end = li; b.off = 0;
+                b.size = head ? (o.irb.Cout2 ? 2 : 1) * SGX_TAIL_CK * F * o.H * o.W : o.outc * F * (o.kind == OP_PW ? o.H * o.W : o.Ho * o.Wo);
+                b.size = (b.size + 3) & ~3;
+                for (int lj = li + 1; lj < T.nl; lj++) if (src_layer[lj] == li) b.end = lj;
+                for (bool moved = true; moved;) {
+                    moved = false;
+                    for (int lj = 0; lj < li; lj++) if (bufs[lj].end >= li && b.off < bufs[lj].off + bufs[lj].size && bufs[lj].off < b.off + b.size) { b.off = bufs[lj].off + bufs[lj].size; moved = true; }
+                }
+                bufs[li] = b; top = std::max(top, b.off + b.size);
+            }
+            if ((size_t)top * 4 > (size_t)160 * 1024) continue;
+            for (int li = 0; li < T.nl; li++) {
+                const Op &o = h->ops[members[li]]; SgxTailLayer &L = T.L[li];
+                const Blob &A = h->blobs[o.in0], &O = h->blobs[o.out];
+                L.src = src_layer[li] < 0 ? -1 : bufs[src_layer[li]].off; L.dst = bufs[li].off;
+                L.in = src_layer[li] < 0 ? A.d : nullptr; L.in_pitch = src_layer[li] < 0 ? A.n : 0;
+                L.out = O.d; L.out_pitch = O.n;
+                L.H = o.H; L.W = o.W;
+                if (o.kind == OP_IRB) {
+                    const SgxIrb &ib = o.irb;
+                    L.kind = SGX_TAIL_HEAD; L.C = ib.Cexp; L.Co = ib.Cout; L.Ho = o.H; L.Wo = o.W; L.S = 1; L.lo = ib.a2lo; L.hi = ib.a2hi;
+                    L.w = ib.wd; L.bias = ib.bd; L.w2T = ib.w2T; L.b2 = ib.b2; L.ld2 = ib.ld2; L.hwc_off = ib.hwc_off;
+                    if (ib.Cout2) {
+                        const Blob &O2 = h->blobs[o.irb_out2_blob];
+                        L.CoB = ib.Cout2; L.wB = ib.wd_b; L.biasB = ib.bd_b; L.w2TB = ib.w2Tb; L.b2B = ib.b2b; L.ld2B = ib.ld2b; L.hwc_offB = ib.hwc_off2; L.outB = O2.d; L.outB_pitch = O2.n;
+                    }
+                } else {
+                    const EpiClass k = classify(o.epi);
+                    L.kind = o.kind == OP_PW ? SGX_TAIL_PW3 : SGX_TAIL_DW; L.C = o.inc; L.Co = o.outc; L.S = o.stride; L.lo = k.lo; L.hi = k.hi;
+                    L.Ho = o.kind == OP_PW ? o.H : o.Ho; L.Wo = o.kind == OP_PW ? o.W : o.Wo;
+                    L.w = o.wt; L.bias = o.bias; L.wS = (const sgx_q4 *)o.wS; L.ldw = o.ldw;
+                }
+                if ((size_t)F * std::max(A.n, O.n) * 4 >= 0x7FFFFFFFull) ok = false;
+            }
+            if (!ok) continue;
+            h->tail = T; h->tail_lds = (size_t)top * 4; h->tail_ops = members;
+            std::sort(h->tail_ops.begin(), h->tail_ops.end());
+        }
+    }
+    if (h->tail_ops.empty()) return SGX_OK;
+    for (int i : h->tail_ops) h->tail_member[i] = 1;
+    h->tail_first = h->tail_ops.front();
+    return sgx_tail_dispatch(h->tail, 1, h->tail_lds, nullptr, true);
+}
+
+static int run_plan(sgx_det *h, size_t first, int batch, sgx_stream_t st)
+{
+    for (size_t i = first; i < h->ops.size(); i++) {
+        int rc = SGX_OK;
+        if ((int)i == h->tail_first) rc = sgx_tail_dispatch(h->tail, batch, h->tail_lds, st, false);
+        if (rc == SGX_OK && !(h->tail_first >= 0 && h->tail_member[i])) rc = run_op(h, h->ops[i], batch, st);
+        if (rc != SGX_OK) return rc;
+    }
+    return SGX_OK;
+}
+
 static int run_first_step(sgx_det *h, const uint8_t *d_img, int pitch, int batch, sgx_stream_t st)
 {
     const int T = h->T;
@@ -1131,7 +1246,7 @@
             if (h->sw.fork_lanes > 1) { if ((rc = capture_forked(h, first, batch, st, h->sw.fork_lanes, &graph)) != SGX_OK) return rc; }
             else {
                 SGX_CHECK_HIP(hipStreamBeginCapture(st, hipStreamCaptureModeThreadLocal));
-                for (size_t i = first; i < h->ops.size(); i++) if ((rc = run_op(h, h->ops[i], batch, st)) != SGX_OK) return abandon_capture(st, rc);
+                if ((rc = run_plan(h, first, batch, st)) != SGX_OK) return abandon_capture(st, rc);
                 SGX_CHECK_HIP(hipStreamEndCapture(st, &graph));
             }
             std::vector<hipGraphExec_t> execs;
@@ -1142,7 +1257,7 @@
         { unsigned &turn = h->graph_turn[batch]; SGX_CHECK_HIP(hipGraphLaunch(it->second[turn % it->second.size()], st)); turn++; }
     } else
 #endif
-    for (size_t i = first; i < h->ops.size(); i++) if ((rc = run_op(h, h->ops[i], batch, st)) != SGX_OK) return rc;
+    if ((rc = run_plan(h, first, batch, st)) != SGX_OK) return rc;
     sgx_prof_end(SGX_K_DET_FWD, st);
     SGX_CHECK_HIP(hipGetLastError());
     if (d_loc) *d_loc = h->blobs[h->loc_blob].d;
@@ -1183,6 +1298,40 @@
     if (i < 0 || i >= nops) return SGX_ERR_INVALID;
     for (int r = 0; r < reps; r++) { const int rc = i == 0 ? run_first_step(h, d_img, pitch, batch, (sgx_stream_t)stream) : run_op(h, h->ops[i - 1 + skip], batch, (sgx_stream_t)stream); if (rc != SGX_OK) return rc; }
     return SGX_OK;
+}
+
+SGX_TAP int sgx_det_debug_tail_steps(const sgx_det *h, int *steps, int cap, int *n)
+{
+    if (!h || !n) return SGX_ERR_INVALID;
+    *n = (int)h->tail_ops.size();
+    if (steps) { if (cap < *n) return SGX_ERR_INVALID; for (int i = 0; i < *n; i++) steps[i] = h->tail_ops[i] + 1 - h->pre_fused; }
+    return SGX_OK;
+}
+SGX_TAP int sgx_det_debug_time_tail(sgx_det *h, int batch, int reps, float *ms)
+{
+    if (!h || !ms || batch < 1 || batch > h->max_batch || reps < 1 || h->tail_first < 0) return SGX_ERR_INVALID;
+#ifndef SGX_EMU
+    hipEvent_t a, b; SGX_CHECK_HIP(hipEventCreate(&a));
+    if (hipEventCreate(&b) != hipSuccess) { (void)hipEventDestroy(a); return SGX_ERR_DEVICE; }
+    float tot = 0.f;
+    auto timed = [&]() -> int {
+        for (int r = 0; r < reps + 1; r++) {
+            SGX_CHECK_HIP(hipEventRecord(a, 0));
+            const int rc = sgx_tail_dispatch(h->tail, batch, h->tail_lds, 0, false);
+            if (rc != SGX_OK) return rc;
+            SGX_CHECK_HIP(hipEventRecord(b, 0)); SGX_CHECK_HIP(hipEventSynchronize(b));
+            float t = 0.f; SGX_CHECK_HIP(hipEventElapsedTime(&t, a, b)); if (r) tot += t;
+        }
+        return SGX_OK;
+    };
+    const int rc = timed();
+    (void)hipEventDestroy(a); (void)hipEventDestroy(b);
+    if (rc != SGX_OK) return rc;
+    *ms = tot / reps;
+    return SGX_OK;
+#else
+    return SGX_ERR_UNSUPPORTED;
+#endif
 }
 
 extern "C" int sgx_det_plan_step(const sgx_det *h, int i, char *buf, int cap)
diff --git a/sg_slam_amd/csrc/sgx_det_tail.h b/sg_slam_amd/csrc/sgx_det_tail.h
--- /dev/null
+++ b/sg_slam_amd/csrc/sgx_det_tail.h
@@ -0,0 +1,264 @@
+#pragma once
+#include "sgx_det_kernels.h"
+#include "sgx_det_bf16.h"
+#include "sgx_lanes.h"
+
+#define SGX_TAIL_MAXL 16
+#define SGX_TAIL_THREADS 512
+#define SGX_TAIL_CK 64
+enum { SGX_TAIL_DW = 0, SGX_TAIL_PW3, SGX_TAIL_HEAD };
+
+struct SgxTailLayer {
+    int kind;
+    int C, Co, H, W, Ho, Wo, S;
+    int src, dst;
+    float lo, hi;
+    const float *in; size_t in_pitch;
+    const float *w, *bias;
+    const sgx_q4 *wS; int ldw;
+    float *out; size_t out_pitch;
+    const float *w2T, *b2; int ld2, hwc_off;
+    const float *wB, *biasB, *w2TB, *b2B; int ld2B, CoB, hwc_offB; float *outB; size_t outB_pitch;
+};
+struct SgxTail { int nl, F, batch; SgxTailLayer L[SGX_TAIL_MAXL]; };
+
+SGX_DEV void sgx_tail_dw(const SgxTailLayer &L, float *Ls, int b0, int nf, int F)
+{
+    const int HWi = L.H * L.W, HWo = L.Ho * L.Wo, NPo = nf * HWo, NSi = F * HWi, NSo = F * HWo;
+    const int nt = (int)blockDim.x, LPC = L.C >= nt ? 1 : nt / L.C, cpp = nt / LPC;
+    const float *X = L.in + (size_t)b0 * L.in_pitch;
+    float *Y = L.out + (size_t)b0 * L.out_pitch;
+    SGX_WAVES_BEGIN(w)
+    const vi gl = v_lane() + w * 64, cl = gl / LPC, p0 = gl - cl * LPC;
+    for (int cb = 0; cb < L.C; cb += cpp) {
+        const vb cok = ((cl + cb) < L.C) & (cl < cpp);
+        const vi c = v_min(cl + cb, vi(L.C - 1));
+        vf wv[9]; const vf bz = v_ld(L.bias, v_u(c) * 4u);
+#pragma unroll
+        for (int t = 0; t < 9; t++) wv[t] = v_ld(L.w, v_u(c * 9 + t) * 4u);
+        for (int i0 = 0; i0 * LPC < NPo; i0 += 4) {
+            vf x[4][9]; vi pp[4], f[4], n[4]; vb live[4];
+#pragma unroll
+            for (int u = 0; u < 4; u++) {
+                const vi pq = p0 + (i0 + u) * LPC;
+                live[u] = cok & (pq < NPo); pp[u] = v_min(pq, vi(NPo - 1));
+                f[u] = pp[u] / HWo; n[u] = pp[u] - f[u] * HWo;
+                const vi oy = n[u] / L.Wo, ox = n[u] - oy * L.Wo;
+#pragma unroll
+                for (int t = 0; t < 9; t++) {
+                    const vi iy = oy * L.S + (t / 3 - 1), ix = ox * L.S + (t % 3 - 1);
+                    const vb ok = (iy >= 0) & (iy < L.H) & (ix >= 0) & (ix < L.W);
+                    const vi pix = v_seli(ok, iy * L.W + ix, vi(0));
+                    const vf v = L.src < 0 ? v_ld(X, v_u(f[u] * (int)L.in_pitch + c * HWi + pix) * 4u) : v_lds_ld(Ls + L.src, c * NSi + f[u] * HWi + pix);
+                    x[u][t] = v_sel(ok, v, vf(0.f));
+                }
+            }
+#pragma unroll
+            for (int u = 0; u < 4; u++) {
+                vf acc = bz;
+#pragma unroll
+                for (int t = 0; t < 9; t++) acc = v_fma(wv[t], x[u][t], acc);
+                const vf r = v_clip(acc, L.lo, L.hi);
+                v_lds_st(Ls + L.dst, c * NSo + pp[u], r);
+                v_st(Y, v_u(f[u] * (int)L.out_pitch + c * HWo + n[u]) * 4u, r, live[u]);
+            }
+        }
+    }
+    SGX_WAVES_END
+}
+
+template <int NPX>
+SGX_DEV void sgx_tail_pw3_task(const SgxTailLayer &L, float *Ls, int t, int m0, int NP, int NS, int HW, float *Y, const vi &l31, const vi &half)
+{
+    const int nks = L.C >> 4;
+    vf16 acc[NPX]; vi pcol[NPX];
+#pragma unroll
+    for (int r = 0; r < 16; r++) {
+        const vf bz = v_ld(L.bias, v_u(half * 4 + (32 * t + (r & 3) + 8 * (r >> 2))) * 4u);
+#pragma unroll
+        for (int m = 0; m < NPX; m++) acc[m][r] = bz;
+    }
+#pragma unroll
+    for (int m = 0; m < NPX; m++) pcol[m] = v_min(l31 + 32 * (m0 + m), vi(NP - 1));
+    vu4 a[4][3];
+#define SGX_TAIL_LDA(s_, d_) do { _Pragma("unroll") for (int q_ = 0; q_ < 3; q_++) a[d_][q_] = v_ldq(L.wS, (half + ((s_) * 3 + q_) * 2) * L.ldw + (l31 + 32 * t)); } while (0)
+    SGX_TAIL_LDA(0, 0); SGX_TAIL_LDA(1, 1); SGX_TAIL_LDA(2, 2);
+    for (int s0 = 0; s0 < nks; s0 += 4) {
+#pragma unroll
+        for (int d = 0; d < 4; d++) {
+            const int s = s0 + d, sn = s + 3 < nks ? s + 3 : nks - 1;
+            SGX_TAIL_LDA(sn, (d + 3) & 3);
+#pragma unroll
+            for (int m = 0; m < NPX; m++) {
+                vf xv[8];
+#pragma unroll
+                for (int j = 0; j < 8; j++) xv[j] = v_lds_ld(Ls + L.src, (half * 8 + (16 * s + j)) * NS + pcol[m]);
+                acc[m] = v_mfma3(a[d][0], a[d][1], a[d][2], v_split3x8(xv), acc[m]);
+            }
+        }
+    }
+#undef SGX_TAIL_LDA
+#pragma unroll
+    for (int m = 0; m < NPX; m++) {
+        const vb live = (l31 + 32 * (m0 + m)) < NP;
+        const vi f = pcol[m] / HW, n = pcol[m] - f * HW;
+#pragma unroll
+        for (int r = 0; r < 16; r++) {
+            const vi row = half * 4 + (32 * t + (r & 3) + 8 * (r >> 2));
+            const vf v = v_clip(acc[m][r], L.lo, L.hi);
+            v_lds_st(Ls + L.dst, row * NS + pcol[m], v);
+            v_st(Y, v_u(f * (int)L.out_pitch + row * HW + n) * 4u, v, live);
+        }
+    }
+}
+
+SGX_DEV void sgx_tail_pw3(const SgxTailLayer &L, float *Ls, int b0, int nf, int F)
+{
+    const int HW = L.H * L.W, NP = nf * HW, NS = F * HW, npx = (NP + 31) >> 5, noc = L.Co >> 5;
+    float *Y = L.out + (size_t)b0 * L.out_pitch;
+    SGX_WAVES_BEGIN(w)
+    const vi lane = v_lane(), l31 = lane & 31, half = lane >> 5;
+    const int nw = (int)blockDim.x >> 6;
+    const bool wide = npx == 2 && noc >= nw;
+    const int ntask = wide ? noc : noc * npx;
+    if (wide) for (int q = w; q < ntask; q += nw) sgx_tail_pw3_task<2>(L, Ls, q, 0, NP, NS, HW, Y, l31, half);
+    else for (int q = w; q < ntask; q += nw) { const int t = q / npx; sgx_tail_pw3_task<1>(L, Ls, t, q - t * npx, NP, NS, HW, Y, l31, half); }
+    SGX_WAVES_END
+}
+
+SGX_DEV void sgx_tail_head(const SgxTailLayer &L, float *Ls, int b0, int nf, int F)
+{
+    constexpr int CK = SGX_TAIL_CK, KS = CK / 2;
+    const int HW = L.H * L.W, NP = nf * HW, NS = F * HW, npx = (NP + 31) >> 5;
+    const int ntA = (L.Co + 31) >> 5, ntB = (L.CoB + 31) >> 5, ntask = (ntA + ntB) * npx, nh = L.CoB ? 2 : 1;
+    float *Sc = Ls + L.dst;
+    SGX_WPRIV_DECL(vf16, acc, 2);
+    SGX_WPRIV_DECL(vf, ar, 2 * KS);
+    SGX_WPRIV_DECL(vf, wd, 2 * 10);
+    const int nt = (int)blockDim.x, LPC = nt / CK;
+#define SGX_TAIL_HEAD_TAPS(c0_) do { const vi c_ = (v_lane() + w * 64) / LPC + (c0_);                                                                  \
+        _Pragma("unroll") for (int hd_ = 0; hd_ < 2; hd_++) if (hd_ < nh) {                                                                             \
+            wd[hd_ * 10 + 9] = v_ld(hd_ ? L.biasB : L.bias, v_u(c_) * 4u);                                                                               \
+            _Pragma("unroll") for (int t_ = 0; t_ < 9; t_++) wd[hd_ * 10 + t_] = v_ld(hd_ ? L.wB : L.w, v_u(c_ * 9 + t_) * 4u); } } while (0)
+    SGX_WAVES_BEGIN(w)
+    SGX_WPRIV_BIND(acc, w); SGX_WPRIV_BIND(wd, w);
+    const vi lane = v_lane(), half = lane >> 5;
+    const int nw = (int)blockDim.x >> 6;
+#pragma unroll
+    for (int k = 0; k < 2; k++) {
+        const int q = w + k * nw;
+        if (q < ntask) {
+            const int tt = q / npx, hb = tt >= ntA ? 1 : 0, tile = hb ? tt - ntA : tt, Cout = hb ? L.CoB : L.Co;
+            const float *bp = hb ? L.b2B : L.b2;
+#pragma unroll
+            for (int r = 0; r < 16; r++) {
+                const vi row = half * 4 + (32 * tile + (r & 3) + 8 * (r >> 2));
+                acc[k][r] = v_sel(row < Cout, v_ld(bp, v_u(v_min(row, vi(Cout - 1))) * 4u), vf(0.f));
+            }
+        }
+    }
+    SGX_TAIL_HEAD_TAPS(0);
+    SGX_WAVES_END
+    for (int c0 = 0; c0 < L.C; c0 += CK) {
+        SGX_WAVES_BEGIN(w)
+        SGX_WPRIV_BIND(ar, w); SGX_WPRIV_BIND(wd, w);
+        const vi lane = v_lane(), l31 = lane & 31, half = lane >> 5;
+        const int nw = (int)blockDim.x >> 6;
+#pragma unroll
+        for (int k = 0; k < 2; k++) {
+            const int q = w + k * nw;
+            if (q < ntask) {
+                const int tt = q / npx, hb = tt >= ntA ? 1 : 0, tile = hb ? tt - ntA : tt, ld = hb ? L.ld2B : L.ld2;
+                const float *wp = hb ? L.w2TB : L.w2T;
+#pragma unroll
+                for (int s = 0; s < KS; s++) ar[k * KS + s] = v_ld(wp, v_u((half + (c0 + 2 * s)) * ld + (l31 + 32 * tile)) * 4u);
+            }
+        }
+        const vi gl = lane + w * 64, cl = gl / LPC, p0 = gl - cl * LPC, c = cl + c0;
+        for (int i0 = 0; i0 * LPC < NP; i0 += 2) {
+#pragma unroll
+            for (int u = 0; u < 2; u++) {
+                const vi pp = v_min(p0 + (i0 + u) * LPC, vi(NP - 1)), f = pp / HW, n = pp - f * HW, oy = n / L.W, ox = n - oy * L.W;
+                vf x[9];
+#pragma unroll
+                for (int t = 0; t < 9; t++) {
+                    const vi iy = oy + (t / 3 - 1), ix = ox + (t % 3 - 1);
+                    const vb ok = (iy >= 0) & (iy < L.H) & (ix >= 0) & (ix < L.W);
+                    x[t] = v_sel(ok, v_lds_ld(Ls + L.src, c * NS + f * HW + v_seli(ok, iy * L.W + ix, vi(0))), vf(0.f));
+                }
+#pragma unroll
+                for (int hd = 0; hd < 2; hd++) if (hd < nh) {
+                    vf dacc = wd[hd * 10 + 9];
+#pragma unroll
+                    for (int t = 0; t < 9; t++) dacc = v_fma(wd[hd * 10 + t], x[t], dacc);
+                    v_lds_st(Sc, cl * NS + pp + hd * CK * NS, v_clip(dacc, L.lo, L.hi));
+                }
+            }
+        }
+        SGX_WAVES_END
+        SGX_SYNC();
+        SGX_WAVES_BEGIN(w)
+        SGX_WPRIV_BIND(acc, w); SGX_WPRIV_BIND(ar, w); SGX_WPRIV_BIND(wd, w);
+        const vi lane = v_lane(), l31 = lane & 31, half = lane >> 5;
+        const int nw = (int)blockDim.x >> 6;
+        if (c0 + CK < L.C) SGX_TAIL_HEAD_TAPS(c0 + CK);
+#pragma unroll
+        for (int k = 0; k < 2; k++) {
+            const int q = w + k * nw;
+            if (q < ntask) {
+                const int tt = q / npx, hb = tt >= ntA ? 1 : 0, m = q - tt * npx;
+                const vi pcol = v_min(l31 + 32 * m, vi(NP - 1));
+#pragma unroll
+                for (int s = 0; s < KS; s++) acc[k] = v_mfma_f32(ar[k * KS + s], v_lds_ld(Sc, (half + 2 * s) * NS + pcol + hb * CK * NS), acc[k]);
+            }
+        }
+        SGX_WAVES_END
+        SGX_SYNC();
+    }
+    SGX_WAVES_BEGIN(w)
+    SGX_WPRIV_BIND(acc, w);
+    const vi lane = v_lane(), l31 = lane & 31, half = lane >> 5;
+    const int nw = (int)blockDim.x >> 6;
+#pragma unroll
+    for (int k = 0; k < 2; k++) {
+        const int q = w + k * nw;
+        if (q < ntask) {
+            const int tt = q / npx, hb = tt >= ntA ? 1 : 0, tile = hb ? tt - ntA : tt, m = q - tt * npx, Cout = hb ? L.CoB : L.Co, off = hb ? L.hwc_offB : L.hwc_off;
+            const size_t pitch = hb ? L.outB_pitch : L.out_pitch;
+            float *Y = (hb ? L.outB : L.out) + (size_t)b0 * pitch;
+            const vi px = l31 + 32 * m, pc = v_min(px, vi(NP - 1)), f = pc / HW, n = pc - f * HW;
+#pragma unroll
+            for (int r = 0; r < 16; r++) {
+                const vi row = half * 4 + (32 * tile + (r & 3) + 8 * (r >> 2));
+                v_st(Y, v_u(f * (int)pitch + n * Cout + v_min(row, vi(Cout - 1)) + off) * 4u, acc[k][r], (px < NP) & (row < Cout));
+            }
+        }
+    }
+    SGX_WAVES_END
+#undef SGX_TAIL_HEAD_TAPS
+}
+
+SGX_KERNEL(SGX_TAIL_THREADS) k_det_tail(SgxTail p)
+{
+    SGX_DYN_LDS(smem);
+    float *Ls = (float *)smem;
+    const int b0 = (int)blockIdx.x * p.F, nf = min(p.F, p.batch - b0);
+    for (int li = 0; li < p.nl; li++) {
+        const SgxTailLayer &L = p.L[li];
+        if (L.kind == SGX_TAIL_DW) sgx_tail_dw(L, Ls, b0, nf, p.F);
+        else if (L.kind == SGX_TAIL_PW3) sgx_tail_pw3(L, Ls, b0, nf, p.F);
+        else sgx_tail_head(L, Ls, b0, nf, p.F);
+        if (L.kind != SGX_TAIL_HEAD) SGX_SYNC();
+    }
+}
+
+static inline bool sgx_tail_dw_ok(int C, int k, int stride, int pad) { return k == 3 && pad == 1 && stride == 2 && C > 0; }
+static inline bool sgx_tail_pw3_ok(int C, int Co, int px) { return (C % 64) == 0 && (Co % 32) == 0 && px <= 64; }
+static inline bool sgx_tail_head_ok(int C, int Co, int CoB, int px, int nwaves) { return (C % SGX_TAIL_CK) == 0 && (64 * nwaves) % SGX_TAIL_CK == 0 && px <= 64 && (((Co + 31) / 32 + (CoB + 31) / 32) * ((px + 31) / 32)) <= 2 * nwaves; }
+static inline int sgx_tail_dispatch(const SgxTail &p, int batch, size_t lds, sgx_stream_t st, bool prepare)
+{
+    if (prepare) return lds <= 160 * 1024 ? sgx_allow_lds(k_det_tail, 160 * 1024) : SGX_ERR_UNSUPPORTED;
+    SgxTail q = p; q.batch = batch;
+    SGX_LAUNCH_DYN(k_det_tail, dim3((unsigned)((batch + p.F - 1) / p.F)), dim3(SGX_TAIL_THREADS), lds, st, q);
+    return SGX_OK;
+}
diff --git a/sg_slam_amd/csrc/sgx_lanes.h b/sg_slam_amd/csrc/sgx_lanes.h
--- a/sg_slam_amd/csrc/sgx_lanes.h
+++ b/sg_slam_amd/csrc/sgx_lanes.h
@@ -43,6 +43,7 @@
     acc = SGX_MFMA_BF16(a0, b.t1, acc); acc = SGX_MFMA_BF16(a1, b.t0, acc);
     return SGX_MFMA_BF16(a0, b.t0, acc);
 }
+SGX_DEV vf16 v_mfma_f32(vf a, vf b, vf16 acc) { return __builtin_amdgcn_mfma_f32_32x32x2f32(a, b, acc, 0, 0, 0); }
 SGX_DEV void v_swap32(vf x, vf y, vf &nx, vf &ny)
 {
     const auto r = __builtin_amdgcn_permlane32_swap(__float_as_uint(x), __float_as_uint(y), false, false);
@@ -126,6 +127,15 @@
     acc = v_mfma1(a0, b.t1, acc); acc = v_mfma1(a1, b.t0, acc);
     return v_mfma1(a0, b.t0, acc);
 }
+static inline vf16 v_mfma_f32(const vf &a, const vf &b, const vf16 &c)
+{
+    vf16 d;
+    for (int half = 0; half < 2; half++) for (int i = 0; i < 32; i++) for (int r = 0; r < 16; r++) {
+        const int row = (r & 3) + 8 * (r >> 2) + 4 * half;
+        d.r[r].v[32 * half + i] = fmaf(a.v[32 + row], b.v[32 + i], fmaf(a.v[row], b.v[i], c.r[r].v[32 * half + i]));
+    }
+    return d;
+}
 static inline void v_swap32(const vf &x, const vf &y, vf &nx, vf &ny)
 {
     vf a, b;
diff --git a/sg_slam_amd/detector.py b/sg_slam_amd/detector.py
--- a/sg_slam_amd/detector.py
+++ b/sg_slam_amd/detector.py
@@ -85,6 +85,21 @@
             out.append(buf.value.decode())
         return out
 
+    def tail_steps(self):
+        n = C.c_int(0)
+        self.lib.check(self.lib.tap('sgx_det_debug_tail_steps')(self.h, None, 0, C.byref(n)))
+        steps = np.zeros(max(n.value, 1), 'i4')
+        self.lib.check(self.lib.tap('sgx_det_debug_tail_steps')(self.h, _vp(steps), len(steps), C.byref(n)))
+        return [int(v) for v in steps[:n.value]]
+
+    def run_step(self, d_img, batch, step, reps=1, stream=None):
+        self.lib.check(self.lib.tap('sgx_det_debug_run_step')(self.h, _vp(d_img), self.width * 3, batch, step, reps, None if stream is None else C.c_void_p(stream)), 'sgx_det_debug_run_step')
+
+    def time_tail(self, batch, reps=5):
+        ms = C.c_float(0)
+        self.lib.check(self.lib.tap('sgx_det_debug_time_tail')(self.h, batch, reps, C.byref(ms)), 'sgx_det_debug_time_tail')
+        return float(ms.value)
+
     def debug_blob(self, name, image=0):
         n = C.c_int(0)
         self.lib.check(self.lib.tap('sgx_det_debug_read_blob')(self.h, name.encode(), image, None, 0, C.byref(n)))
```

New measurement: 29830, median of 6. 1.02x the previous value.
